# zichunhao/lgn-autoencoder

Hardware: AMD Instinct MI355X
Metric: jets/sec fwd+bwd, 30-particle maxdim=2 bs=512 (higher is better)
Workload: dtype f64

## Files before the change

### include/lgn_amd.h

```cpp
#ifndef LGN_AMD_H
#define LGN_AMD_H

#include <stddef.h>
#include <stdint.h>

#ifdef __cplusplus
extern "C" {
#endif

#define LGN_AMD_ABI_VERSION 19

int lgn_abi_version(void);
const char* lgn_last_error(void);

int lgn_level_fwd_f64(int B, int N, int C, int CO, int decoder,
                      const double* s_in, const double* v_in, const double* p, const uint8_t* mask,
                      const double* ra, const double* rb, const double* rc,
                      const double* w0, const double* b0, const double* w1, const double* b1,
                      const double* wm0, const double* wm1,
                      double* ag0, double* ag1, double* s_out, double* v_out, void* stream);

int lgn_level_bwd_partial_rows(int B, int N, int decoder, int* rows_mix, int* rows_rad);
int lgn_level_rad_partial_len(int C, int decoder);
int lgn_level_jet_split(int B, int N);

int lgn_level_bwd_f64(int B, int N, int C, int CO, int decoder,
                      const double* s_in, const double* v_in, const double* p, const uint8_t* mask,
                      const double* ra, const double* rb, const double* rc,
                      const double* w0, const double* b0, const double* w1, const double* b1,
                      const double* wm0, const double* wm1, const double* ag0, const double* ag1,
                      const double* g_s_out, const double* g_v_out,
                      double* g_ag, double* g_s_in, double* g_v_in, double* g_p,
                      double* part_mix, double* part_rad, void* stream);

int lgn_cg_product_fwd_f64(int R, int N, int C, int D1, int D2, int DO, int mode, int nnz, const int* row_ptr, const int* col,
                           const double* coef, const double* x1, const double* x2, double* out, void* stream);
int lgn_cg_product_bwd_f64(int R, int N, int C, int D1, int D2, int DO, int mode, int nnz, const int* row_ptr, const int* col,
                           const double* coef, const double* x1, const double* x2, const double* g_out, double* g_x1, double* g_x2,
                           void* stream);

int lgn_reduce_partials_f64(const double* part, int rows, int n, double* out, int accumulate, void* stream);

int lgn_radial_finalize_f64(const double* tot, int C, const double* ra, const double* rb, const double* rc,
                            const double* w0, const double* w1,
                            double* g_a, double* g_b, double* g_c,
                            double* g_w0, double* g_b0, double* g_w1, double* g_b1, void* stream);

#define LGN_ACT_LEAKYRELU 0
#define LGN_ACT_RELU 1
#define LGN_ACT_ELU 2
#define LGN_ACT_SIGMOID 3
#define LGN_ACT_LOGSIGMOID 4
#define LGN_ACT_ATAN 5
#define LGN_ACT_COUNT 6
int lgn_cgmlp_fwd_f64(int M, int C, int H, int nlin, int activation, const double* const* w, const double* const* b,
                      const double* s_in, double* s_out, void* stream);
int lgn_cgmlp_partial_rows(int M, int H);
int lgn_cgmlp_bwd_f64(int M, int C, int H, int nlin, int activation, const double* const* w, const double* const* b,
                      const double* s_in, const double* g_out, double* g_in, double* part, int psize, void* stream);

int lgn_mixreps_fwd_f64(int rows, int Cin, int Cout, int d, const double* w, const double* x, double* y, void* stream);
int lgn_mixreps_partial_rows(int rows);
int lgn_mixreps_bwd_f64(int rows, int Cin, int Cout, int d, const double* w, const double* x, const double* g_y,
                        double* g_x, double* part, void* stream);

int lgn_moments_fwd_f64(int B, int N, int C, int Q, int decoder, const double* X, const double* p, const uint8_t* mask,
                        const double* ra, const double* rb, const double* rc, const double* w0, const double* b0,
                        const double* w1, const double* b1, double* U, void* stream);
long long lgn_moments_scratch_doubles(int B, int N, int C, int decoder);
int lgn_moments_bwd_f64(int B, int N, int C, int Q, int decoder, const double* X, const double* p, const uint8_t* mask,
                        const double* ra, const double* rb, const double* rc, const double* w0, const double* b0,
                        const double* w1, const double* b1, const double* gU, double* gX, double* g_p,
                        double* part_rad, double* scratch, void* stream);

typedef struct lgn_local_tables {
  int n_rows, n_out, n_w;
  int n_terms, n_u, n_x;
  int n_units, static_kind;
  const int *row_ptr, *t_type, *t_a, *t_b;
  const double* t_coef;
  const int *out_dim, *out_nblk, *out_row0, *out_q0, *out_w0;
  const int *u_ptr, *u_row;
  const double* u_coef;
  const int *x_ptr, *x_row, *x_other;
  const double* x_coef;
  int h_out_w0[8];
} lgn_local_tables;

int lgn_local_fwd_f64(int nodes, int C, int CO, int Q, int Qout, const lgn_local_tables* t, const double* X, const double* U,
                      const double* wcat, double* out, void* stream);
int lgn_local_partial_rows(int nodes);
int lgn_local_bwd_f64(int nodes, int C, int CO, int Q, int Qout, const lgn_local_tables* t, const double* X, const double* U,
                      const double* wcat, const double* g_out, double* gU, double* gX, double* part, void* stream);

long long lgn_local_static_packed_doubles(int kind, int C, int CO);
int lgn_local_bwd_static_f64(int kind, int nodes, int C, int CO, const double* XT, const double* UT, const double* wcat,
                             const int* w0, double* wpacked, const double* goT, double* gUT, double* gXT, double* part,
                             double* gpacked, double* g_wcat, void* stream);
int lgn_local_fwd_static_f64(int kind, int nodes, int C, int CO, const double* XT, const double* UT, const double* wcat,
                             const int* w0, double* wpacked, double* outT, double* s_copy, int q_s, void* stream);

typedef struct lgn_net_desc {
  int B, N;
  int n_levels;
  int enc_channels[5];
  int dec_channels[5];
  int tau_s, tau_v;
  int mlp_hidden_mul;
  int mlp_nlin;
  int tau_v_in;
  const lgn_local_tables* enc_tables[4];
  const lgn_local_tables* dec_tables[4];
  int enc_Q[5], enc_qs[5], enc_qv[5];
  int dec_Q[5], dec_qs[5], dec_qv[5];
  int flags;
  int activation;
  int n_in_scalars;
  int latent_pool;
  int dec_N;
  int get_real;
  double jet_loss_scale;
} lgn_net_desc;
#define LGN_REAL_SUM 0
#define LGN_REAL_REAL 1
#define LGN_REAL_IMAG 2
#define LGN_REAL_MEAN 3
#define LGN_REAL_NORM 4
#define LGN_LOSS_CHAMFER 0
#define LGN_LOSS_MSE 1
#define LGN_LOSS_HUNGARIAN 2
typedef struct lgn_loss_desc {
  int kind;
  int abs_coord;
  int polar_coord;
  double scale;
} lgn_loss_desc;
#define LGN_POOL_MIN 0
#define LGN_POOL_MAX 1
#define LGN_POOL_MEAN 2
#define LGN_POOL_MIX 3
#define LGN_POOL(n, avg, o0, o1, o2, o3) ((n) | ((avg) << 3) | ((o0) << 4) | ((o1) << 6) | ((o2) << 8) | ((o3) << 10))
#define LGN_NET_NO_STATIC 1
#define LGN_NET_DEC_PAIRWISE 2
#define LGN_NET_LEVEL_V2 4
#define LGN_NET_MLP_V1 8
#define LGN_NET_MOMENTS_V1 16
#define LGN_NET_BWD_ORDERED 64
#define LGN_NET_DEC_UNFUSED 256
#define LGN_NET_MOMENTS_SPLIT 512
#define LGN_NET_MLP_BWD1 1024
#define LGN_NET_SPLIT_TAIL 128

#define LGN_LDS_LIMIT (160 * 1024)
long long lgn_encoder_end_lds_bytes(int N, int C0, int K, int CL, int Ts, int Tv, int pool);
long long lgn_decoder_end_lds_bytes(int N, int C0, int Tin, int CL);
long long lgn_junction_lds_bytes(int N, int CL, int Ts, int Tv, int pool, int C0);

int lgn_step_param_slots(const lgn_net_desc* d, int decoder);
long long lgn_step_workspace_doubles(const lgn_net_desc* d);
int lgn_step_fwd_bwd_f64(const lgn_net_desc* d, const double* params, double* grads, long long n_params,
                         const int64_t* enc_off, const int64_t* dec_off, const double* p4, const double* target,
                         const uint8_t* mask, const double* in_scalars, double* workspace, long long workspace_doubles,
                         double* recon, double* loss_part, const lgn_loss_desc* loss, int* assignment ,
                         int* status , void* stream);
#define LGN_FINALIZE_SCRATCH 2048
int lgn_step_finalize_f64(double* params, double* grads, long long n_params, const double* loss_part, int n_loss,
                          double l1_lambda, double* adam_m, double* adam_v, long long* step_dev,
                          double lr, double beta1, double beta2, double eps, int do_adam, double* loss_out, void* stream);
int lgn_step_train_f64(const lgn_net_desc* d, double* params, double* grads, long long n_params, const int64_t* enc_off,
                       const int64_t* dec_off, const double* p4, const double* target, const uint8_t* mask, const double* in_scalars,
                       double* workspace, long long workspace_doubles, double* recon, double* loss_part, int n_loss, double l1_lambda,
                       double* adam_m, double* adam_v, long long* step_dev, double lr, double beta1, double beta2, double eps,
                       int do_adam, double* loss_out, const lgn_loss_desc* loss, int* assignment ,
                       int* status , void* stream);

#define LGN_OPT_ADAM 0
#define LGN_OPT_RMSPROP 1
typedef struct {
  int kind;
  double l1_lambda, l2_lambda, lr, eps;
  double beta1, beta2;
  double alpha, momentum;
} lgn_optim_desc;
#define LGN_FINALIZE_OPT_SCRATCH 4096
int lgn_step_finalize_opt_f64(double* params, double* grads, long long n_params, const double* loss_part, int n_loss,
                              const lgn_optim_desc* opt, double* state_m, double* state_v, long long* step_dev, int do_step,
                              double* loss_out, void* stream);
int lgn_step_train_opt_f64(const lgn_net_desc* d, double* params, double* grads, long long n_params, const int64_t* enc_off,
                           const int64_t* dec_off, const double* p4, const double* target, const uint8_t* mask,
                           const double* in_scalars, double* workspace, long long workspace_doubles, double* recon,
                           double* loss_part, int n_loss, const lgn_optim_desc* opt, double* state_m, double* state_v,
                           long long* step_dev, int do_step, double* loss_out, const lgn_loss_desc* loss,
                           int* assignment , int* status , void* stream);

long long lgn_eval_workspace_doubles(const lgn_net_desc* d);
int lgn_step_eval_f64(const lgn_net_desc* d, const double* params, const int64_t* enc_off, const int64_t* dec_off,
                      const double* p4_scaled, const double* p4_target, const uint8_t* mask, const double* in_scalars,
                      double* workspace, long long workspace_doubles, double* recon_real, double* lat_s ,
                      double* lat_v , double* loss_part, double* loss_out, const lgn_loss_desc* loss,
                      int* assignment , int* status , void* stream);

long long lgn_net_workspace_doubles(const lgn_net_desc* d, int decoder, int which);
int lgn_encoder_fwd_f64(const lgn_net_desc* d, const double* params, const int64_t* off, const double* p4, const uint8_t* mask,
                        const double* in_scalars, double* act, long long act_doubles, double* lat_s, double* lat_v, void* stream);
int lgn_encoder_bwd_f64(const lgn_net_desc* d, const double* params, double* grads, long long n_params, const int64_t* off,
                        const double* p4, const uint8_t* mask, const double* in_scalars, const double* act, long long act_doubles,
                        const double* g_lat_s, const double* g_lat_v, double* scratch, long long scratch_doubles, void* stream);
int lgn_decoder_fwd_f64(const lgn_net_desc* d, const double* params, const int64_t* off, const double* lat_v, double* act,
                        long long act_doubles, double* recon, void* stream);
int lgn_decoder_bwd_f64(const lgn_net_desc* d, const double* params, double* grads, long long n_params, const int64_t* off,
                        const double* lat_v, const double* act, long long act_doubles, const double* g_recon, double* g_lat_v,
                        double* scratch, long long scratch_doubles, void* stream);

int lgn_chamfer_f64(int B, int N, int M, const double* x, const double* y, int jet_features, double* loss_part, double* gx, double* gy,
                    void* stream);

#define LGN_ANOMALY_NMAX 192
#define LGN_ANOMALY_NSCORES 21
#define LGN_ANOMALY_ALL 0x1FFFFF
#define LGN_ANOMALY_HUNGARIAN 0x403E0
#define LGN_ANOMALY_NO_HUNGARIAN (LGN_ANOMALY_ALL & ~LGN_ANOMALY_HUNGARIAN)
int lgn_anomaly_scores_f64(const double* recons, const double* target, const double* recons_n, const double* target_n, int B, int N,
                           int score_mask, double* scores, int* col4row , int* status, void* stream);

#define LGN_ROC_TILE 2048
#define LGN_ROC_MAX_COLS 65535
#define LGN_ROC_NONFINITE 1
#define LGN_ROC_SINGLE_CLASS 2
#define LGN_ROC_BAD_LABEL 4
#define LGN_ROC_NAN 8
long long lgn_roc_workspace_bytes(long long M, int K);
int lgn_roc_auc_f64(const double* scores, long long M, int ld, int K, const double* labels, double* fpr, double* tpr,
                    double* thresholds, int* length, double* auc, int* flipped, int* status, void* workspace,
// ... 113 lines not shown
```

### lgn-autoencoder_amd/csrc/api.hip

```cpp
#include "net.hpp"

using namespace lgn;

extern "C" {

int lgn_level_fwd_f64(int B, int N, int C, int CO, int decoder, const double* s_in, const double* v_in, const double* p,
                      const uint8_t* mask, const double* ra, const double* rb, const double* rc, const double* w0,
                      const double* b0, const double* w1, const double* b1, const double* wm0, const double* wm1,
                      double* ag0, double* ag1, double* s_out, double* v_out, void* stream) {
  LGN_CHECK_ARG(s_in && v_in && p && b0 && b1 && wm0 && wm1 && ag0 && ag1 && s_out && v_out, "level_fwd: null pointer");
  LGN_CHECK_ARG(decoder || (mask && ra && rb && rc && w0 && w1), "level_fwd: encoder needs mask and radial parameters");
  LevelArgs<double> a{B, N, C, CO, s_in, v_in, p, mask, ra, rb, rc, w0, b0, w1, b1, wm0, wm1, ag0, ag1, s_out, v_out};
  a.flags = level_flags_from_env();
  return level_fwd_dispatch<double>(a, decoder, (hipStream_t)stream);
}

int lgn_level_bwd_partial_rows(int B, int N, int decoder, int* rows_mix, int* rows_rad) {
  LGN_CHECK_ARG(B > 0 && N > 0 && rows_mix && rows_rad, "level_bwd_partial_rows: bad arguments");
  level_bwd_partial_rows(B, N, decoder, level_flags_from_env(), rows_mix, rows_rad);
  return 0;
}

int lgn_level_rad_partial_len(int C, int decoder) { return rad_partial_size(C, decoder != 0); }
int lgn_level_jet_split(int B, int N) { return N <= 40 ? level_jet_split(B, N) : 1; }

int lgn_level_bwd_f64(int B, int N, int C, int CO, int decoder, const double* s_in, const double* v_in, const double* p,
                      const uint8_t* mask, const double* ra, const double* rb, const double* rc, const double* w0,
                      const double* b0, const double* w1, const double* b1, const double* wm0, const double* wm1,
                      const double* ag0, const double* ag1, const double* g_s_out, const double* g_v_out, double* g_ag,
                      double* g_s_in, double* g_v_in, double* g_p, double* part_mix, double* part_rad, void* stream) {
  LGN_CHECK_ARG(s_in && v_in && p && b0 && b1 && wm0 && wm1 && ag0 && ag1 && g_s_out && g_v_out && g_ag && g_s_in &&
                    g_v_in && part_mix && part_rad, "level_bwd: null pointer");
  LGN_CHECK_ARG(decoder ? (g_p != nullptr) : (mask && ra && rb && rc && w0 && w1), "level_bwd: missing decoder g_p / encoder radial parameters");
  LevelBwdArgs<double> a{B, N, C, CO, s_in, v_in, p, mask, ra, rb, rc, w0, b0, w1, b1, wm0, wm1, ag0, ag1,
                         g_s_out, g_v_out, g_ag, g_s_in, g_v_in, g_p, part_mix, part_rad};
  a.flags = level_flags_from_env();
  return level_bwd_dispatch<double>(a, decoder, (hipStream_t)stream);
}

int lgn_cg_product_fwd_f64(int R, int N, int C, int D1, int D2, int DO, int mode, int nnz, const int* row_ptr, const int* col,
                           const double* coef, const double* x1, const double* x2, double* out, void* stream) {
  return cg_product_fwd(R, N, C, D1, D2, DO, mode, nnz, row_ptr, col, coef, x1, x2, out, (hipStream_t)stream);
}
int lgn_cg_product_bwd_f64(int R, int N, int C, int D1, int D2, int DO, int mode, int nnz, const int* row_ptr, const int* col,
                           const double* coef, const double* x1, const double* x2, const double* g_out, double* g_x1, double* g_x2,
                           void* stream) {
  return cg_product_bwd(R, N, C, D1, D2, DO, mode, nnz, row_ptr, col, coef, x1, x2, g_out, g_x1, g_x2, (hipStream_t)stream);
}

int lgn_reduce_partials_f64(const double* part, int rows, int n, double* out, int accumulate, void* stream) {
  LGN_CHECK_ARG(part && out && rows > 0 && n >= 0, "reduce_partials: bad arguments");
  return reduce_partials<double>(part, rows, n, out, accumulate, (hipStream_t)stream);
}

int lgn_radial_finalize_f64(const double* tot, int C, const double* ra, const double* rb, const double* rc, const double* w0,
                            const double* w1, double* g_a, double* g_b, double* g_c, double* g_w0, double* g_b0,
                            double* g_w1, double* g_b1, void* stream) {
  LGN_CHECK_ARG(tot && ra && rb && rc && w0 && w1 && g_a && g_b && g_c && g_w0 && g_b0 && g_w1 && g_b1 && C >= 1 && C <= 8,
                "radial_finalize: bad arguments");
  return rad_finalize<double>(tot, C, ra, rb, rc, w0, w1, g_a, g_b, g_c, g_w0, g_b0, g_w1, g_b1, (hipStream_t)stream);
}

static int fill_mlp(MlpArgs<double>& a, int M, int C, int H, int nlin, int activation, const double* const* w, const double* const* b) {
  LGN_CHECK_ARG(nlin >= 1 && nlin <= MLP_MAX_LIN && w && b, "cgmlp: bad layer list (nlin=%d)", nlin);
  a.M = M; a.C = C; a.H = H; a.nlin = nlin; a.act = activation;
  for (int l = 0; l < MLP_MAX_LIN; ++l) {
    a.w[l] = l < nlin ? w[l] : nullptr;
    a.b[l] = l < nlin ? b[l] : nullptr;
    if (l < nlin) LGN_CHECK_ARG(w[l] && b[l], "cgmlp: null weight pointer for layer %d", l);
  }
  return 0;
}

int lgn_cgmlp_fwd_f64(int M, int C, int H, int nlin, int activation, const double* const* w, const double* const* b,
                      const double* s_in, double* s_out, void* stream) {
  MlpArgs<double> a{};
  if (int rc = fill_mlp(a, M, C, H, nlin, activation, w, b)) return rc;
  LGN_CHECK_ARG(s_in && s_out, "cgmlp_fwd: null pointer");
  a.s_in = s_in; a.s_out = s_out;
  a.flags = level_flags_from_env();
  return mlp_dispatch<double>(a, false, (hipStream_t)stream);
}

int lgn_cgmlp_partial_rows(int M, int H) { return mlp_partial_rows(M, H); }

int lgn_cgmlp_bwd_f64(int M, int C, int H, int nlin, int activation, const double* const* w, const double* const* b,
                      const double* s_in, const double* g_out, double* g_in, double* part, int psize, void* stream) {
  MlpArgs<double> a{};
  if (int rc = fill_mlp(a, M, C, H, nlin, activation, w, b)) return rc;
  LGN_CHECK_ARG(s_in && g_out && g_in && part, "cgmlp_bwd: null pointer");
  a.s_in = s_in; a.g_out = g_out; a.g_in = g_in; a.part = part; a.psize = psize;
  a.flags = level_flags_from_env();
  return mlp_dispatch<double>(a, true, (hipStream_t)stream);
}

int lgn_mixreps_fwd_f64(int rows, int Cin, int Cout, int d, const double* w, const double* x, double* y, void* stream) {
  LGN_CHECK_ARG(w && x && y, "mixreps_fwd: null pointer");
// ... 253 lines not shown
```

### lgn-autoencoder_amd/csrc/api_common.cpp

```cpp
#include <stdarg.h>
#include <stdlib.h>

#include "level.hpp"
#include "../../include/lgn_amd.h"

namespace lgn {
static thread_local char g_err[512] = "";
void set_error(const char* fmt, ...) {
  va_list ap;
  va_start(ap, fmt);
  vsnprintf(g_err, sizeof(g_err), fmt, ap);
  va_end(ap);
}
int level_flags_from_env() {
  auto on = [](const char* name) { const char* e = getenv(name); return e && e[0] == '1'; };
  return (on("LGN_AMD_DEC_PAIRWISE") ? LVL_DEC_PAIRWISE : 0) | (on("LGN_AMD_LEVEL_V2") ? LVL_LEVEL_V2 : 0) |
         (on("LGN_AMD_MOMENTS_V1") ? LVL_MOMENTS_V1 : 0) | (on("LGN_AMD_MLP_V1") ? LVL_MLP_V1 : 0) | (on("LGN_AMD_BWD_ORDERED") ? LVL_BWD_ORDERED : 0) |
         (on("LGN_AMD_MOMENTS_SPLIT") ? LVL_MOMENTS_SPLIT : 0) | (on("LGN_AMD_MLP_BWD1") ? LVL_MLP_BWD1 : 0);
}
static_assert(LVL_DEC_PAIRWISE == LGN_NET_DEC_PAIRWISE && LVL_LEVEL_V2 == LGN_NET_LEVEL_V2 && LVL_MOMENTS_V1 == LGN_NET_MOMENTS_V1 &&
                  LVL_MLP_V1 == LGN_NET_MLP_V1 && LVL_MLP_BWD1 == LGN_NET_MLP_BWD1 &&
                  LVL_BWD_ORDERED == LGN_NET_BWD_ORDERED && LVL_MOMENTS_SPLIT == LGN_NET_MOMENTS_SPLIT, "LVL_* and LGN_NET_* are the same bits");
}

extern "C" {
const char* lgn_last_error(void) { return lgn::g_err; }
int lgn_abi_version(void) { return LGN_AMD_ABI_VERSION; }
}
```

### lgn-autoencoder_amd/csrc/level.hpp

```cpp
#pragma once
#include "common.hpp"

namespace lgn {

constexpr int LVL_DEC_PAIRWISE = 2;
constexpr int LVL_LEVEL_V2 = 4;
constexpr int LVL_MLP_V1 = 8;
constexpr int LVL_MOMENTS_V1 = 16;
constexpr int LVL_MLP_BWD1 = 1024;
constexpr int LVL_MOMENTS_SPLIT = 512;
constexpr int LVL_BWD_ORDERED = 64;
int level_flags_from_env();

template <typename T>
struct LevelArgs {
  int B, N, C, CO;
  const T* s_in;
  const T* v_in;
  const T* p;
  const uint8_t* mask;
  const T *ra, *rb, *rc, *w0, *b0, *w1, *b1;
  const T *wm0, *wm1;
  T* ag0;
  T* ag1;
  T* s_out;
  T* v_out;
  const T* in_w0 = nullptr;
  const T* in_w1 = nullptr;
  T* in_s = nullptr;
  T* in_v = nullptr;
  T* z1 = nullptr;
  size_t z1n = 0;
  T* z2 = nullptr;
  size_t z2n = 0;
  const T* loss_wo1 = nullptr;
  const T* loss_target = nullptr;
  T loss_scale = T(1);
  int loss_real = 0;
  T loss_jscale = T(0);
  T* loss_recon = nullptr;
  T* loss_part = nullptr;
  T* loss_gv = nullptr;
  T* loss_wpart = nullptr;
  int flags = 0;
};

template <typename T>
struct LevelBwdArgs {
  int B, N, C, CO;
  const T *s_in, *v_in, *p;
  const uint8_t* mask;
  const T *ra, *rb, *rc, *w0, *b0, *w1, *b1;
  const T *wm0, *wm1;
  const T *ag0, *ag1;
  const T* g_s_out;
  const T* g_v_out;
  T* g_ag;
  T* g_s_in;
  T* g_v_in;
  T* g_p;
  T* part_mix;
  T* part_rad;
  T* part_in0 = nullptr;
  int flags = 0;
};

__host__ __device__ constexpr int node_stride(int C) { return 10 * C + 4; }

__host__ __device__ constexpr int rad_partial_size(int C, bool dec) {
  return dec ? 2 * C : (2 * 4 * C * NB + 8 * C);
}

inline int level_jet_split(int B, int N) {
  const int groups = (N + 3) / 4;
  int s = 1;
  while (s * 2 <= groups && B * s * 2 <= 512) s *= 2;
  return s;
}

}
```

### lgn-autoencoder_amd/csrc/level_bwd3.hip

```cpp
#include "level_dev.hpp"
#include "ops.hpp"
#include "wave_sum.hpp"

namespace lgn {

typedef double v4d __attribute__((ext_vector_type(4)));

namespace {
__device__ __forceinline__ double dppq(double v, int xor2) {
  int lo = __double2loint(v), hi = __double2hiint(v);
  if (xor2) {
    lo = __builtin_amdgcn_mov_dpp(lo, 0x4E, 0xF, 0xF, true);
    hi = __builtin_amdgcn_mov_dpp(hi, 0x4E, 0xF, 0xF, true);
  } else {
    lo = __builtin_amdgcn_mov_dpp(lo, 0xB1, 0xF, 0xF, true);
    hi = __builtin_amdgcn_mov_dpp(hi, 0xB1, 0xF, 0xF, true);
  }
  return __hiloint2double(hi, lo);
}
__device__ __forceinline__ double quad_sum(double v) {
  v += dppq(v, 0);
  v += dppq(v, 1);
  return v;
}
__device__ __forceinline__ double fast_rcp(double u) {
  double r = __builtin_amdgcn_rcp(u);
  double e = __builtin_fma(-u, r, 1.0);
  r = __builtin_fma(r, e, r);
  e = __builtin_fma(-u, r, 1.0);
  return __builtin_fma(r, e, r);
}
__device__ __forceinline__ void wave_sync() {
  __builtin_amdgcn_fence(__ATOMIC_RELEASE, "workgroup");
  __builtin_amdgcn_wave_barrier();
  __builtin_amdgcn_fence(__ATOMIC_ACQUIRE, "workgroup");
}
template <int C> struct GA3 {
  static constexpr int A3 = 0, A4 = 2 * C, A1 = 4 * C, A2 = 12 * C, SIZE = 20 * C + 2;
};
constexpr int TS = 18;
LGN_STAMP_DECL
}
LGN_STAMP_READER(lgn_debug_stamps_bwd3)

template <int C, bool DEC, int NWV = 4>
struct Bwd3 {
  static constexpr int BLK = 64 * NWV;
  static constexpr int NG = (C + 3) / 4;
  static constexpr int NS = node_stride(C);
  static constexpr int PS = DEC ? 8 : 4;
  static constexpr int TRSZ = DEC ? NWV * 64 : (NWV * (NG + 3) * 16 * TS > NWV * 64 * NG * 12 ? NWV * (NG + 3) * 16 * TS : NWV * 64 * NG * 12);
  static constexpr int MIXP = BLK / (5 * C) < 16 ? BLK / (5 * C) : 16;
  __host__ __device__ static size_t scratch(int N, int CO) {
    size_t p1 = (size_t)N * 10 * CO + 4 * CO * 5 * C + (size_t)N * 20 * C;
    const size_t red = (size_t)MIXP * CO * 5 * C * 4;
    if (red > p1) p1 = red;
    return p1 > (size_t)TRSZ ? p1 : (size_t)TRSZ;
  }
  static constexpr int SMS = 52;
  static constexpr int SEPSZ = DEC ? SMS * C : 0;
  static size_t smem(int N, int CO) {
    return sizeof(double) * ((((size_t)N * NS + 1) & ~size_t(1)) + (size_t)N * (20 * C + 2) + (size_t)N * 10 * C + (size_t)N * PS +
                             scratch(N, CO) + SEPSZ) + N + 16;
  }
};

template <int C, bool DEC, bool SEP, int NWV, bool SYM = false>
__global__ __launch_bounds__(64 * NWV) __attribute__((amdgpu_waves_per_eu(C <= 4 || DEC ? 2 : 1, C <= 4 || DEC ? 2 : 1))) void level_bwd3_kernel(LevelBwdArgs<double> a) {
  static_assert(!SYM || !DEC, "the symmetric sweep is the encoder's");
  using F = Bwd3<C, DEC, NWV>;
  constexpr int BLK = F::BLK;
  using G = GA3<C>;
  constexpr int NG = F::NG, NS = F::NS, PS = F::PS, K = 5 * C;
  const int N = a.N, B = a.B, CO = a.CO;
  const int b = blockIdx.x, tid = threadIdx.x, lane = tid & 63, wave = tid >> 6;
  const int ngroups = (N + 3) >> 2, gper = (ngroups + (int)gridDim.y - 1) / (int)gridDim.y;
  const int glo = min(ngroups, (int)blockIdx.y * gper), ghi = min(ngroups, glo + gper);
  const int nlo = min(N, 4 * glo), nhi = min(N, 4 * ghi);
  const size_t prow = (size_t)b * gridDim.y + blockIdx.y;

  extern __shared__ __align__(16) unsigned char smem_raw[];
  double* nd = reinterpret_cast<double*>(smem_raw);
  double* ga = nd + ((N * NS + 1) & ~1);
  double* gd = ga + N * G::SIZE;
  double* pj = gd + N * 10 * C;
  double* tr = pj + N * PS;
  double* go = tr;
  double* wm = go + N * 10 * CO;
  double* agl = wm + 4 * CO * K;
  double* sm = tr + F::scratch(N, CO);
  uint8_t* mk = reinterpret_cast<uint8_t*>(sm + F::SEPSZ);

  STAMP(0);
  {
    const size_t plo = (size_t)B * N * CO, pa = (size_t)B * N * 2 * C;
    JetRegs<double> jr;
    load_jet_issue<double, C, DEC>(a.s_in, a.v_in, a.p, a.mask, B, N, b, jr);
    const int eg = tid < N * CO ? tid : 0, ea_ = tid < N * 2 * C ? tid : 0, ew = tid < 2 * CO * K ? tid : 0;
    const size_t ig = (size_t)b * N * CO + eg, ia = (size_t)b * N * 2 * C + ea_;
    double rg[10], ra[10];
    rg[0] = a.g_s_out[ig];
    rg[1] = a.g_s_out[plo + ig];
    ra[0] = a.ag0[ia];
    ra[1] = a.ag0[pa + ia];
#pragma unroll
    for (int m = 0; m < 4; ++m) {
      rg[2 + m] = a.g_v_out[ig * 4 + m];
      rg[6 + m] = a.g_v_out[plo * 4 + ig * 4 + m];
      ra[2 + m] = a.ag1[ia * 4 + m];
      ra[6 + m] = a.ag1[(pa + ia) * 4 + m];
    }
    const double w0v = a.wm0[ew], w1v = a.wm1[ew];
    load_jet_commit<double, C, DEC>(a.s_in, a.v_in, a.p, a.mask, B, N, b, jr, nd, pj, mk);
    if (tid < N * CO) {
#pragma unroll
      for (int m = 0; m < 10; ++m) go[tid * 10 + m] = rg[m];
    }
    if (tid < N * 2 * C) {
#pragma unroll
      for (int m = 0; m < 10; ++m) agl[tid * 10 + m] = ra[m];
    }
    if (tid < 2 * CO * K) {
      wm[tid] = w0v;
      wm[2 * CO * K + tid] = w1v;
    }
    for (int e = tid + BLK; e < 2 * CO * K; e += BLK) {
      wm[e] = a.wm0[e];
      wm[2 * CO * K + e] = a.wm1[e];
    }
    for (int e = tid + BLK; e < N * CO; e += BLK) {
      const size_t idx = (size_t)b * N * CO + e;
      double* g = go + e * 10;
      g[0] = a.g_s_out[idx];
      g[1] = a.g_s_out[plo + idx];
#pragma unroll
      for (int m = 0; m < 4; ++m) {
        g[2 + m] = a.g_v_out[idx * 4 + m];
        g[6 + m] = a.g_v_out[plo * 4 + idx * 4 + m];
      }
    }
    for (int e = tid + BLK; e < N * 2 * C; e += BLK) {
      const size_t ea = (size_t)b * N * 2 * C + e;
      double* x = agl + e * 10;
      x[0] = a.ag0[ea];
      x[1] = a.ag0[pa + ea];
#pragma unroll
      for (int m = 0; m < 4; ++m) {
        x[2 + m] = a.ag1[ea * 4 + m];
        x[6 + m] = a.ag1[(pa + ea) * 4 + m];
      }
    }
  }
  __syncthreads();
  STAMP(1);

  {
    const int half = tid >= BLK / 2;
    for (int e = half ? tid - BLK / 2 : tid; e < N * C; e += BLK / 2) {
// ... 268 lines not shown
          const double* q = sm + c * F::SMS;
          const double* ni = nd + n * NS + c * 10;
          const cx<double> R1 = {a.b1[c], a.b1[c]};
          const cx<double> S = {q[0], q[1]}, SG3 = {q[22], q[23]};
          const cx<double> VSt = {sg * q[2 + 2 * mp], sg * q[3 + 2 * mp]};
          const cx<double> vt = {sg * ni[2 + mp], sg * ni[6 + mp]};
          const cx<double> g2 = {gi[G::A2 + (c * 4 + m) * 2], gi[G::A2 + (c * 4 + m) * 2 + 1]};
          const cx<double> g3 = {0.5 * gi[G::A3 + 2 * c], 0.5 * gi[G::A3 + 2 * c + 1]};
          cx<double> t = cmulc(g2, S);
          cfmac(t, g3, VSt);
          const cx<double> t2 = cmulc(cx<double>{q[32 + 2 * m], q[33 + 2 * m]}, cx<double>{ni[0], ni[1]});
          t.r -= t2.r;  t.i -= t2.i;
          const cx<double> t3 = cmulc(SG3, vt);
          t.r -= t3.r;  t.i -= t3.i;
          cfmac(acc, t, R1);
        }
        a.g_p[((size_t)b * N + n) * 4 + m] += acc.r;
        a.g_p[plp + ((size_t)b * N + n) * 4 + m] += acc.i;
      }
    }
    if (tid < 2 * C) {
      const int lin = tid / C, c = tid - lin * C;
      const double* q = sm + c * F::SMS;
      const cx<double> S = {q[0], q[1]};
      double* part = a.part_rad + (size_t)blockIdx.x * rad_partial_size(C, true);
      if (lin == 0) {
        cx<double> E0 = cmulc(cx<double>{q[20], q[21]}, S);
#pragma unroll
        for (int m = 0; m < 4; ++m) cfmac(E0, cx<double>{q[24 + 2 * m], q[25 + 2 * m]}, cx<double>{q[2 + 2 * m], q[3 + 2 * m]});
        part[tid] = (E0.r + E0.i) + (E0.i - E0.r);
      } else {
        cx<double> VS[4], VSt[4];
#pragma unroll
        for (int m = 0; m < 4; ++m) VS[m] = {q[2 + 2 * m], q[3 + 2 * m]};
        metric_perm(VS, VSt);
        cx<double> E1 = cmulc(cx<double>{q[40], q[41]}, S);
        cx<double> neg = cmulc(cx<double>{q[22], q[23]}, cx<double>{q[18], q[19]});
#pragma unroll
        for (int m = 0; m < 4; ++m) {
          cfmac(neg, cx<double>{q[32 + 2 * m], q[33 + 2 * m]}, cx<double>{q[10 + 2 * m], q[11 + 2 * m]});
          cfmac(E1, cx<double>{q[42 + 2 * m], q[43 + 2 * m]}, VSt[m]);
        }
        part[tid] = (E1.r - neg.r) + (E1.i - neg.i);
      }
    }
    STAMP(7);
    return;
  }

  STAMP(3);
  const int pr = lane & 15, cg = lane >> 4;
  const int tj = pr >> 2, ti = pr & 3;
  double ak[5], bk[5], ck2[5], wf[NG][5], bias[NG][4];
  if (!DEC) {
#pragma unroll
    for (int s = 0; s < 5; ++s) {
      const int k = 4 * s + cg;
      ak[s] = a.ra[k];
      bk[s] = a.rb[k];
      const double c = a.rc[k];
      ck2[s] = c * c;
    }
#pragma unroll
    for (int g = 0; g < NG; ++g) {
      const int rr = lane & 15, q = rr >> 2, ch = 4 * g + (rr & 3);
      const double* w = (q >> 1) ? a.w1 : a.w0;
#pragma unroll
      for (int s = 0; s < 5; ++s) wf[g][s] = ch < C ? w[(2 * ch + (q & 1)) * NB + 4 * s + cg] : 0.0;
    }
  }
#pragma unroll
  for (int g = 0; g < NG; ++g) {
    const int ch = 4 * g + cg;
#pragma unroll
    for (int q = 0; q < 4; ++q) {
      const double* bb = (q >> 1) ? a.b1 : a.b0;
      bias[g][q] = ch < C ? (DEC ? bb[ch] : bb[2 * ch + (q & 1)]) : 0.0;
    }
  }
  STAMP(4);
  __syncthreads();
  STAMP(5);

  double* trw = tr + wave * (NG + 3) * 16 * TS;
  v4d T[NG][3];
  double dB0[NG], dB1[NG];
#pragma unroll
  for (int g = 0; g < NG; ++g) {
    dB0[g] = dB1[g] = 0.0;
#pragma unroll
    for (int t = 0; t < 3; ++t) T[g][t] = v4d{0, 0, 0, 0};
  }
  const size_t pls = (size_t)B * N * C;
  double in0[NG][4];
#pragma unroll
  for (int g = 0; g < NG; ++g) in0[g][0] = in0[g][1] = in0[g][2] = in0[g][3] = 0.0;
  const int gcount = ghi - glo;
  const int rs = (!SYM && !DEC && NWV == 4 && gcount >= 1 && gcount <= 2) ? NWV / gcount : 1;
  const int rpart = rs > 1 ? wave % rs : 0;
  const int ntl = (N + 3) >> 2, i0lo = rs > 1 ? 4 * (rpart * ntl / rs) : 0, i0hi = rs > 1 ? min(N, 4 * ((rpart + 1) * ntl / rs)) : N;
  for (int u = 0;; ++u) {
    int rg;
    if constexpr (SYM) {
      const int p = wave + NWV * (u >> 1);
      if (p >= (ngroups + 1) >> 1) break;
      rg = (u & 1) ? ngroups - 1 - p : p;
      if ((u & 1) && rg == p) continue;
    } else if (rs > 1) {
      if (u > 0) break;
      rg = glo + wave / rs;
    } else {
      rg = glo + wave + NWV * u;
      if (rg >= ghi) break;
    }
    const int j = rg * 4 + tj;
    const bool jok = j < N;
    const int jj = jok ? j : N - 1;
    double pme[PS];
#pragma unroll
    for (int m = 0; m < PS; ++m) pme[m] = pj[jj * PS + m];
    const bool mj = DEC ? false : (mk[jj] != 0);
    cx<double> Gs[NG], Gv[NG][4], Gq[4];
    cx<double> sj[NG], vj[NG][4], vtj[NG][4];
    cx<double> dvj[NG], svj[NG];
#pragma unroll
    for (int g = 0; g < NG; ++g) {
      Gs[g] = {0, 0};
#pragma unroll
      for (int m = 0; m < 4; ++m) Gv[g][m] = {0, 0};
      const int ch = 4 * g + cg, cs = ch < C ? ch : 0;
      const double* nj = nd + jj * NS + cs * 10;
      sj[g] = {nj[0], nj[1]};
#pragma unroll
      for (int m = 0; m < 4; ++m) vj[g][m] = {nj[2 + m], nj[6 + m]};
      metric_perm(vj[g], vtj[g]);
      dvj[g] = {vj[g][3].r - vj[g][1].r, vj[g][3].i - vj[g][1].i};
      svj[g] = {vj[g][1].r + vj[g][3].r, vj[g][1].i + vj[g][3].i};
    }
#pragma unroll
    for (int m = 0; m < 4; ++m) Gq[m] = {0, 0};

    for (int i0 = i0lo; i0 < i0hi; i0 += 4) {
      if (rg == glo && i0 < 32) STAMP(16 + (i0 >> 2) * 4);
      const int kind = SYM ? ((i0 >> 2) < rg ? 2 : ((i0 >> 2) == rg ? 1 : 0)) : 1;
      const int i = i0 + ti;
      const bool ok = jok && i < N;
      const int ii = i < N ? i : N - 1;
      const double* pii = pj + ii * PS;
      cx<double> q[4];
      v4d R[NG];
      double rho[5], an = 0.0;
      double qd0 = 0.0, qd3 = 0.0, qa = 0.0, qb = 0.0;
      bool on = false;
      if (DEC) {
#pragma unroll
        for (int m = 0; m < 4; ++m) q[m] = {pii[m] - pme[m], pii[4 + m] - pme[4 + m]};
#pragma unroll
        for (int g = 0; g < NG; ++g) R[g] = v4d{bias[g][0], bias[g][1], bias[g][2], bias[g][3]};
      } else {
        const double d0 = pii[0] - pme[0], d1 = pii[1] - pme[1], d2 = pii[2] - pme[2], d3 = pii[3] - pme[3];
        const double q0 = d0 * d0, q1 = d1 * d1, q2 = d2 * d2, q3 = d3 * d3;
        const double nsq = (2.0 * q0 - (((q0 + q1) + q2) + q3)) + 1e-16;
        an = fabs(nsq);
        on = ok && mj && (mk[ii] != 0) && (nsq != 0.0);
        const double h = rsqrt2<double>();
        q[0] = {d0, 0.0};
        q[1] = {d1 * h, -d2 * h};
        q[2] = {d3, 0.0};
        q[3] = {-d1 * h, -d2 * h};
        qd0 = d0;  qd3 = d3;  qa = d1 * h;  qb = d2 * h;
        double beta[5] = {0.0, 0.0, 0.0, 0.0, 0.0};
#pragma unroll
        for (int s = 0; s < 5; ++s) rho[s] = 0.0;
        if (on) {
#pragma unroll
          for (int s = 0; s < 5; ++s) beta[s] = 1.0 + ck2[s] * an;
          rcp5(beta, rho);
#pragma unroll
          for (int s = 0; s < 5; ++s) beta[s] = __builtin_fma(bk[s], rho[s], ak[s]);
        }
#pragma unroll
        for (int g = 0; g < NG; ++g) {
          R[g] = v4d{bias[g][0], bias[g][1], bias[g][2], bias[g][3]};
#pragma unroll
          for (int s = 0; s < 5; ++s) R[g] = __builtin_amdgcn_mfma_f64_16x16x4f64(wf[g][s], beta[s], R[g], 0, 0, 0);
        }
        if (kind != 0) {
          double* xb = trw + NG * 16 * TS;
#pragma unroll
          for (int s = 0; s < 5; ++s) {
            const double x2 = an * rho[s] * rho[s];
            if (s < 4) {
              xb[pr * TS + 4 * s + cg] = rho[s];
              xb[16 * TS + pr * TS + 4 * s + cg] = x2;
            } else {
              xb[32 * TS + pr * TS + cg] = rho[s];
              xb[32 * TS + pr * TS + 4 + cg] = x2;
            }
          }
          xb[32 * TS + pr * TS + 8 + 2 * cg] = cg == 0 ? (on ? 1.0 : 0.0) : 0.0;
          xb[32 * TS + pr * TS + 9 + 2 * cg] = cg == 0 ? (ok ? 1.0 : 0.0) : 0.0;
        }
      }
      if (rg == glo && i0 < 32) STAMP(17 + (i0 >> 2) * 4);
      const double* gi = ga + ii * G::SIZE;
#pragma unroll
      for (int g = 0; g < NG; ++g) {
        const int ch = 4 * g + cg;
        double G0r = 0, G0i = 0, G1r = 0, G1i = 0;
        if (ok && ch < C) {
          const cx<double> R0 = {R[g][0], R[g][1]}, R1 = {R[g][2], R[g][3]};
          const cx<double> e0 = {R0.r - R0.i, R0.r + R0.i};
          const cx<double> gA3 = {0.5 * gi[G::A3 + 2 * ch], 0.5 * gi[G::A3 + 2 * ch + 1]};
          const cx<double> gA4 = {gi[G::A4 + 2 * ch], gi[G::A4 + 2 * ch + 1]};
          cx<double> gA1[4], gA2[4];
#pragma unroll
          for (int m = 0; m < 4; ++m) {
            gA1[m] = {gi[G::A1 + (ch * 4 + m) * 2], gi[G::A1 + (ch * 4 + m) * 2 + 1]};
            gA2[m] = {gi[G::A2 + (ch * 4 + m) * 2], gi[G::A2 + (ch * 4 + m) * 2 + 1]};
          }
          cfmac(Gs[g], gA4, e0);
          cx<double> ge0 = cmulc(gA4, sj[g]);
          cx<double> gR1;
          if (!DEC) {
            const cx<double> dg = {gA2[1].r - gA2[3].r, gA2[1].i - gA2[3].i}, sg = {gA2[1].r + gA2[3].r, gA2[1].i + gA2[3].i};
// ... 237 lines not shown
  if constexpr (!DEC) {
    if (a.part_in0) {
#pragma unroll
      for (int g = 0; g < NG; ++g)
#pragma unroll
        for (int k = 0; k < 4; ++k) {
          double x = in0[g][k];
          x += shfl_xor(x, 4);
          x += shfl_xor(x, 8);
          if (pr == 0 && 4 * g + cg < C) in0l[wave][4 * g + cg][k] = x;
        }
    }
  }

  STAMP(8);
  __syncthreads();
  STAMP(9);
  if constexpr (!DEC) {
    if (a.part_in0 && tid < 4 * C) {
      const int k = tid / C, c = tid - k * C;
      double s = 0;
#pragma unroll
      for (int w = 0; w < NWV; ++w) s += in0l[w][c][k];
      a.part_in0[prow * 4 * C + k * C + c] = s;
    }
  }
  double* part = a.part_rad + prow * rad_partial_size(C, DEC);
  if (DEC) {
    double* red = tr;
#pragma unroll
    for (int g = 0; g < NG; ++g) {
      double x0 = dB0[g], x1 = dB1[g];
      for (int m = 1; m < 16; m <<= 1) { x0 += shfl_xor(x0, m); x1 += shfl_xor(x1, m); }
      if (pr == 0) {
        red[(wave * NG + g) * 8 + cg] = x0;
        red[(wave * NG + g) * 8 + 4 + cg] = x1;
      }
    }
    __syncthreads();
    if (tid < 2 * C) {
      const int lin = tid / C, ch = tid - lin * C, g = ch >> 2, c4 = ch & 3;
      double s = 0;
      for (int w = 0; w < NWV; ++w) s += red[(w * NG + g) * 8 + lin * 4 + c4];
      part[tid] = s;
    }
  } else {
    double* red = tr;
    {
      double* mine = red + (size_t)(wave * 64 + lane) * NG * 12;
#pragma unroll
      for (int g = 0; g < NG; ++g)
#pragma unroll
        for (int t = 0; t < 3; ++t)
#pragma unroll
          for (int q = 0; q < 4; ++q) mine[(g * 3 + t) * 4 + q] = T[g][t][q];
    }
    __syncthreads();
    const int wq = __builtin_amdgcn_readfirstlane(wave);
    if (wq < 4) {
      constexpr int R = 4 * C;
      const int col = lane & 15;
#pragma unroll
      for (int g = 0; g < NG; ++g) {
        const int ch = 4 * g + cg;
#pragma unroll
        for (int t = 0; t < 3; ++t)
#pragma unroll
          for (int q = 0; q < 4; ++q) {
            if (q != wq) continue;
            const int e = (g * 3 + t) * 4 + q;
            double v = (red[(size_t)(0 * 64 + lane) * NG * 12 + e] + red[(size_t)(1 * 64 + lane) * NG * 12 + e]) +
                       (red[(size_t)(2 * 64 + lane) * NG * 12 + e] + red[(size_t)(3 * 64 + lane) * NG * 12 + e]);
            if (NWV == 8)
              v += (red[(size_t)(4 * 64 + lane) * NG * 12 + e] + red[(size_t)(5 * 64 + lane) * NG * 12 + e]) +
                   (red[(size_t)(6 * 64 + lane) * NG * 12 + e] + red[(size_t)(7 * 64 + lane) * NG * 12 + e]);
            if (ch >= C) continue;
            const int r = (q >> 1) * 2 * C + 2 * ch + (q & 1);
            if (t == 0) part[r * NB + col] = v;
            else if (t == 1) part[R * NB + r * NB + col] = v;
            else {
              if (col < 4) part[r * NB + 16 + col] = v;
              else if (col < 8) part[R * NB + r * NB + 16 + (col - 4)] = v;
              else if (col == 8) part[2 * R * NB + r] = v;
              else if (col == 9) part[2 * R * NB + R + r] = v;
            }
          }
      }
    }
  }
  STAMP(10);
}

bool level_bwd3_fits(int N) { return N <= 40; }

template <int C, bool DEC, bool SEP, int NWV>
static int launch_bwd3_w(const LevelBwdArgs<double>& a, int split, hipStream_t stream) {
  size_t smem = Bwd3<C, DEC, NWV>::smem(a.N, a.CO);
  LGN_CHECK_ARG(smem <= 160 * 1024, "level_bwd: N=%d C=%d needs %zu B of LDS", a.N, a.C, smem);
  LGN_CHECK_ARG(a.CO <= 8, "level_bwd: C_out=%d unsupported (1..8)", a.CO);
  auto kern = level_bwd3_kernel<C, DEC, SEP, NWV>;
  if constexpr (!DEC && C <= 4) {
    if (split == 1 && !(a.flags & LVL_BWD_ORDERED)) kern = level_bwd3_kernel<C, DEC, SEP, NWV, true>;
  }
  if (smem > 64 * 1024) (void)hipFuncSetAttribute(reinterpret_cast<const void*>(kern), hipFuncAttributeMaxDynamicSharedMemorySize, (int)smem);
  hipLaunchKernelGGL(kern, dim3(a.B, split), dim3(64 * NWV), smem, stream, a);
  LGN_CHECK_LAUNCH();
  return 0;
}
template <int C, bool DEC, bool SEP>
static int launch_bwd3(const LevelBwdArgs<double>& a, hipStream_t stream) {
  return launch_bwd3_w<C, DEC, SEP, 4>(a, SEP ? 1 : level_jet_split(a.B, a.N), stream);
}

int level_bwd3_dispatch(const LevelBwdArgs<double>& a, int decoder, hipStream_t stream) {
  const bool pairwise = (a.flags & LVL_DEC_PAIRWISE) != 0;
#define LGN_CASE(CC)                                                                \
  case CC:                                                                          \
    if (!decoder) return launch_bwd3<CC, false, false>(a, stream);                  \
    return pairwise ? launch_bwd3<CC, true, false>(a, stream) : launch_bwd3<CC, true, true>(a, stream);
  switch (a.C) {
#ifdef LGN_DEV_ONLY_C4
    LGN_CASE(4)
#else
    LGN_CASE(1) LGN_CASE(2) LGN_CASE(3) LGN_CASE(4) LGN_CASE(5) LGN_CASE(6) LGN_CASE(7) LGN_CASE(8)
#endif
    default: set_error("level_bwd: C_in=%d unsupported (1..8)", a.C); return -1;
  }
#undef LGN_CASE
}

}
```

### lgn-autoencoder_amd/csrc/level_fwd2.hip

```cpp
#include "level_dev.hpp"
#include "net_dev.hpp"
#include "ops.hpp"
#include "wave_sum.hpp"

namespace lgn {

typedef double v4d __attribute__((ext_vector_type(4)));
LGN_STAMP_DECL
LGN_STAMP_READER(lgn_debug_stamps_fwd2)

__device__ __forceinline__ double dpp_quad(double v, int ctrl_is_xor2) {
  int lo = __double2loint(v), hi = __double2hiint(v);
  if (ctrl_is_xor2) {
    lo = __builtin_amdgcn_mov_dpp(lo, 0x4E, 0xF, 0xF, true);
    hi = __builtin_amdgcn_mov_dpp(hi, 0x4E, 0xF, 0xF, true);
  } else {
    lo = __builtin_amdgcn_mov_dpp(lo, 0xB1, 0xF, 0xF, true);
    hi = __builtin_amdgcn_mov_dpp(hi, 0xB1, 0xF, 0xF, true);
  }
  return __hiloint2double(hi, lo);
}
__device__ __forceinline__ double quad_sum(double v) {
  v += dpp_quad(v, 0);
  v += dpp_quad(v, 1);
  return v;
}

__device__ __forceinline__ double fast_rcp(double u) {
  double r = __builtin_amdgcn_rcp(u);
  double e = __builtin_fma(-u, r, 1.0);
  r = __builtin_fma(r, e, r);
  e = __builtin_fma(-u, r, 1.0);
  return __builtin_fma(r, e, r);
}

template <int C, bool DEC>
struct Fwd2 {
  static constexpr int NG = (C + 3) / 4;
  static constexpr int NS = node_stride(C);
  static constexpr int PS = DEC ? 8 : 4;
  static constexpr int AGS = 20 * C;
  static constexpr int A3 = 0, A4 = 2 * C, A1 = 4 * C, A2 = 12 * C;
};

template <int C, bool DEC, bool SEP, bool TRAIN>
__global__ __launch_bounds__(2 * BLOCK) void level_fwd2_kernel(LevelArgs<double> a, int chunk) {
  using F = Fwd2<C, DEC>;
  constexpr int NG = F::NG;
  const int N = a.N, B = a.B, CO = a.CO;
  const int b = blockIdx.x, tid = threadIdx.x, lane = tid & 63, wave = tid >> 6;
  const int nthr = blockDim.x, nw = nthr >> 6;

  extern __shared__ __align__(16) unsigned char smem_raw[];
  double* nd = reinterpret_cast<double*>(smem_raw);
  double* pj = nd + ((N * F::NS + 1) & ~1);
  double* wm = pj + N * F::PS;
  double* agl = wm + 4 * CO * 5 * C;
  double* sums = agl + chunk * F::AGS;
  uint8_t* mk = reinterpret_cast<uint8_t*>(sums + 20 * C);

  STAMP(0);
  if (!DEC && a.in_w0) {
    {
      const size_t wg = (size_t)blockIdx.y * gridDim.x + blockIdx.x, stride = (size_t)gridDim.x * gridDim.y * nthr;
      for (size_t e = wg * nthr + tid; e < a.z1n; e += stride) a.z1[e] = 0.0;
      for (size_t e = wg * nthr + tid; e < a.z2n; e += stride) a.z2[e] = 0.0;
    }
    const double* p0 = a.p + (size_t)b * N * 4;
    const size_t plane_s = (size_t)B * N * C;
    const int nw2 = 2 * CO * 5 * C;
    for (int e = tid; e < N * 4; e += nthr) pj[e] = p0[e];
    for (int e = tid; e < N; e += nthr) mk[e] = a.mask[(size_t)b * N + e];
    for (int e = tid; e < nw2; e += nthr) {
      wm[e] = a.wm0[e];
      wm[nw2 + e] = a.wm1[e];
    }
    for (int e = tid; e < N * C; e += nthr) {
      const int j = e / C, c = e - j * C;
      const double* p = p0 + j * 4;
      const double pe = p[0], px = p[1], py = p[2], pz = p[3];
      const double q0 = pe * pe, q1 = px * px, q2 = py * py, q3 = pz * pz;
      const double mass = sqrt(fabs(2.0 * q0 - (((q0 + q1) + q2) + q3)));
      constexpr double H = 0.70710678118654752440084436210484903928;
      const cx<double> q[4] = {{pe, 0.0}, {px * H, -py * H}, {pz, 0.0}, {-px * H, -py * H}};
      const double w0r = a.in_w0[c], w0i = a.in_w0[C + c];
      const cx<double> w1 = {a.in_w1[c], a.in_w1[C + c]};
      double* d = nd + j * F::NS + c * 10;
      d[0] = w0r * mass;
      d[1] = w0i * mass;
#pragma unroll
      for (int m = 0; m < 4; ++m) {
        const cx<double> r = cmul(w1, q[m]);
        d[2 + m] = r.r;
        d[6 + m] = r.i;
      }
      if (blockIdx.y == 0) {
        const size_t ge = (size_t)b * N * C + e;
        a.in_s[ge] = d[0];
        a.in_s[plane_s + ge] = d[1];
#pragma unroll
        for (int m = 0; m < 4; ++m) {
          a.in_v[ge * 4 + m] = d[2 + m];
          a.in_v[plane_s * 4 + ge * 4 + m] = d[6 + m];
        }
      }
    }
  } else {
    JetRegs<double> jr;
    load_jet_issue<double, C, DEC>(a.s_in, a.v_in, a.p, a.mask, B, N, b, jr);
    const int nw2 = 2 * CO * 5 * C, ew = tid < nw2 ? tid : 0;
    const double w0v = a.wm0[ew], w1v = a.wm1[ew];
    load_jet_commit<double, C, DEC>(a.s_in, a.v_in, a.p, a.mask, B, N, b, jr, nd, pj, mk);
    if (tid < nw2) {
      wm[tid] = w0v;
      wm[nw2 + tid] = w1v;
    }
    for (int e = tid + nthr; e < nw2; e += nthr) {
      wm[e] = a.wm0[e];
      wm[nw2 + e] = a.wm1[e];
    }
  }

  const int pr = lane & 15, cg = lane >> 4;
  const int ti = pr >> 2, tj = pr & 3;
  double ak[5], bk[5], ck2[5];
  double wf[NG][5];
  double bias[NG][4];
  if (!DEC) {
#pragma unroll
    for (int s = 0; s < 5; ++s) {
      const int k = 4 * s + cg;
      ak[s] = a.ra[k];
      bk[s] = a.rb[k];
      const double c = a.rc[k];
      ck2[s] = c * c;
    }
#pragma unroll
    for (int g = 0; g < NG; ++g) {
      const int rr = lane & 15, q = rr >> 2, ch = 4 * g + (rr & 3);
      const double* w = (q >> 1) ? a.w1 : a.w0;
#pragma unroll
      for (int s = 0; s < 5; ++s) wf[g][s] = ch < C ? w[(2 * ch + (q & 1)) * NB + 4 * s + cg] : 0.0;
    }
  }
#pragma unroll
  for (int g = 0; g < NG; ++g) {
    const int ch = 4 * g + cg;
#pragma unroll
    for (int q = 0; q < 4; ++q) {
      const double* bb = (q >> 1) ? a.b1 : a.b0;
      bias[g][q] = ch < C ? (DEC ? bb[ch] : bb[2 * ch + (q & 1)]) : 0.0;
    }
  }
  __syncthreads();
  STAMP(1);

  if constexpr (DEC && SEP) {
    if (tid < 64) {
      const int k = tid & 7, part = tid >> 3;
      double mean = 0.0;
      for (int n = part; n < N; n += 8) mean += pj[n * 8 + k];
      mean += shfl_xor(mean, 8);
      mean += shfl_xor(mean, 16);
      mean += shfl_xor(mean, 32);
      if (part == 0) sums[k] = mean / N;
    }
    __syncthreads();
    for (int e = tid; e < N * 8; e += nthr) pj[e] -= sums[e & 7];
    __syncthreads();
#define LGN_PUT(k, val)                                           \
  do {                                                            \
    if ((k) < 12) a0[(k) < 12 ? (k) : 0] += (val);                \
    else a1[(k) >= 12 ? (k) - 12 : 0] += (val);                   \
  } while (0)
    for (int c = wave; c < C; c += nw) {
      double a0[12], a1[8];
#pragma unroll
      for (int k = 0; k < 12; ++k) a0[k] = 0.0;
#pragma unroll
      for (int k = 0; k < 8; ++k) a1[k] = 0.0;
      for (int n = lane; n < N; n += 64) {
        const double* ni = nd + n * F::NS + c * 10;
        const double* pn = pj + n * 8;
        const cx<double> sn = {ni[0], ni[1]};
        cx<double> v[4], pc[4];
#pragma unroll
        for (int m = 0; m < 4; ++m) {
          v[m] = {ni[2 + m], ni[6 + m]};
          pc[m] = {pn[m], pn[4 + m]};
        }
        LGN_PUT(0, sn.r);  LGN_PUT(1, sn.i);
#pragma unroll
        for (int m = 0; m < 4; ++m) {
          LGN_PUT(2 + 2 * m, v[m].r);  LGN_PUT(3 + 2 * m, v[m].i);
          const cx<double> sp = cmul(sn, pc[m]);
          LGN_PUT(10 + 2 * m, sp.r);  LGN_PUT(11 + 2 * m, sp.i);
        }
        const cx<double> vp = bil2(v, pc);
        LGN_PUT(18, vp.r);  LGN_PUT(19, vp.i);
      }
      wave_sum_store<12>(a0, sums + c * 20, lane);
      wave_sum_store<8>(a1, sums + c * 20 + 12, lane);
    }
#undef LGN_PUT
    __syncthreads();
  }

  const int ngroups = (N + 3) >> 2, gper = (ngroups + (int)gridDim.y - 1) / (int)gridDim.y;
  const int rlo = min(N, 4 * (int)blockIdx.y * gper), rhi = min(N, rlo + 4 * gper);
  auto catmix = [&](int c0, int c1) {
    constexpr int K = 5 * C;
    const int nr = c1 - c0;
    const size_t plo = (size_t)B * N * CO;
    if (wave == 0) {
      for (int rl = lane; rl < nr; rl += 64) {
        const int r = c0 + rl;
        const double* st = agl + rl * F::AGS;
        const double* ni = nd + r * F::NS;
        cx<double> x[K];
#pragma unroll
        for (int c = 0; c < C; ++c) {
          const cx<double> sc = {ni[c * 10], ni[c * 10 + 1]};
          cx<double> v[4];
#pragma unroll
          for (int mm = 0; mm < 4; ++mm) v[mm] = {ni[c * 10 + 2 + mm], ni[c * 10 + 6 + mm]};
          cx<double> vv = bil2(v, v);
          vv.r *= 0.5;  vv.i *= 0.5;
          x[c] = {st[F::A3 + 2 * c], st[F::A3 + 2 * c + 1]};
          x[C + c] = {st[F::A4 + 2 * c], st[F::A4 + 2 * c + 1]};
          x[2 * C + c] = sc;
          x[3 * C + c] = vv;
          x[4 * C + c] = cmul(sc, sc);
        }
#pragma unroll 2
        for (int o = 0; o < CO; ++o) {
          const double* wr = wm + (0 * CO + o) * K;
          const double* wi = wm + (1 * CO + o) * K;
          cx<double> acc = {0, 0};
#pragma unroll
          for (int k = 0; k < K; ++k) cfma(acc, cx<double>{wr[k], wi[k]}, x[k]);
          const size_t e = ((size_t)b * N + r) * CO + o;
          a.s_out[e] = acc.r;
          a.s_out[plo + e] = acc.i;
        }
      }
    } else {
      for (int it = lane + 64 * (wave - 1); it < nr * 4; it += 64 * (nw - 1)) {
        const int rl = it >> 2, m = it & 3, r = c0 + rl;
        const double* st = agl + rl * F::AGS;
        const double* ni = nd + r * F::NS;
        cx<double> x[K];
#pragma unroll
        for (int c = 0; c < C; ++c) {
          const cx<double> sc = {ni[c * 10], ni[c * 10 + 1]};
          const cx<double> v = {ni[c * 10 + 2 + m], ni[c * 10 + 6 + m]};
          x[c] = {st[F::A1 + (c * 4 + m) * 2], st[F::A1 + (c * 4 + m) * 2 + 1]};
          x[C + c] = {st[F::A2 + (c * 4 + m) * 2], st[F::A2 + (c * 4 + m) * 2 + 1]};
          x[2 * C + c] = v;
          x[3 * C + c] = x[4 * C + c] = cmul(v, sc);
        }
#pragma unroll 2
        for (int o = 0; o < CO; ++o) {
          const double* wr = wm + 2 * CO * K + (0 * CO + o) * K;
          const double* wi = wm + 2 * CO * K + (1 * CO + o) * K;
          cx<double> acc = {0, 0};
#pragma unroll
          for (int k = 0; k < K; ++k) cfma(acc, cx<double>{wr[k], wi[k]}, x[k]);
          const size_t e = ((size_t)b * N + r) * CO + o;
          a.v_out[e * 4 + m] = acc.r;
          a.v_out[plo * 4 + e * 4 + m] = acc.i;
        }
      }
    }
    };
  for (int c0 = rlo; c0 < rhi; c0 += chunk) {
  const int c1 = min(rhi, c0 + chunk);
  if constexpr (DEC && SEP) {
    for (int e = tid; e < (c1 - c0) * C; e += nthr) {
      const int rl = e / C, c = e - rl * C, n = c0 + rl;
      const double* sm = sums + c * 20;
      const double* pn = pj + n * 8;
      const cx<double> R0 = {a.b0[c], a.b0[c]}, R1 = {a.b1[c], a.b1[c]};
      const cx<double> e0 = {R0.r - R0.i, R0.r + R0.i};
      const cx<double> S = {sm[0], sm[1]};
      cx<double> VS[4], pc[4];
#pragma unroll
      for (int m = 0; m < 4; ++m) {
        VS[m] = {sm[2 + 2 * m], sm[3 + 2 * m]};
        pc[m] = {pn[m], pn[4 + m]};
      }
      double* st = agl + rl * F::AGS;
      const cx<double> a4 = cmul(S, e0);
// ... 43 lines not shown
      int jj;
      bool ok;
    };
    auto prep = [&](int j0, Tile& T) {
      const int j = j0 + tj;
      T.ok = iok && j < N;
      T.jj = j < N ? j : N - 1;
      const double* pjj = pj + T.jj * F::PS;
      if (DEC) {
#pragma unroll
        for (int m = 0; m < 4; ++m) T.q[m] = {pi[m] - pjj[m], pi[4 + m] - pjj[4 + m]};
#pragma unroll
        for (int g = 0; g < NG; ++g) T.R[g] = v4d{bias[g][0], bias[g][1], bias[g][2], bias[g][3]};
      } else {
        const double d0 = pi[0] - pjj[0], d1 = pi[1] - pjj[1], d2 = pi[2] - pjj[2], d3 = pi[3] - pjj[3];
        const double q0 = d0 * d0, q1 = d1 * d1, q2 = d2 * d2, q3 = d3 * d3;
        const double nsq = (2.0 * q0 - (((q0 + q1) + q2) + q3)) + 1e-16;
        const double an = fabs(nsq);
        const bool on = T.ok && mi && (mk[T.jj] != 0) && (nsq != 0.0);
        const double h = rsqrt2<double>();
        T.qd0 = d0;  T.qd3 = d3;  T.qa = d1 * h;  T.qb = d2 * h;
        double beta[5] = {0.0, 0.0, 0.0, 0.0, 0.0};
        if (on) {
#pragma unroll
          for (int s = 0; s < 5; ++s) beta[s] = 1.0 + ck2[s] * an;
          double rho5[5];
          rcp5(beta, rho5);
#pragma unroll
          for (int s = 0; s < 5; ++s) beta[s] = __builtin_fma(bk[s], rho5[s], ak[s]);
        }
#pragma unroll
        for (int g = 0; g < NG; ++g) {
          T.R[g] = v4d{bias[g][0], bias[g][1], bias[g][2], bias[g][3]};
#pragma unroll
          for (int s = 0; s < 5; ++s) T.R[g] = __builtin_amdgcn_mfma_f64_16x16x4f64(wf[g][s], beta[s], T.R[g], 0, 0, 0);
        }
      }
    };
    auto agg = [&](const Tile& T) {
      if (T.ok) {
        const double* nj = nd + T.jj * F::NS;
#pragma unroll
        for (int g = 0; g < NG; ++g) {
          const int ch = 4 * g + cg;
          if (ch < C) {
            const cx<double> R0 = {T.R[g][0], T.R[g][1]}, R1 = {T.R[g][2], T.R[g][3]};
            const cx<double> e0 = {R0.r - R0.i, R0.r + R0.i};
            const cx<double> sj = {nj[ch * 10], nj[ch * 10 + 1]};
            cx<double> vj[4];
#pragma unroll
            for (int m = 0; m < 4; ++m) {
              vj[m] = {nj[ch * 10 + 2 + m], nj[ch * 10 + 6 + m]};
              cfma(A1[g][m], vj[m], e0);
            }
            cfma(A4[g], sj, e0);
            if (!DEC) {
              const double qd0 = T.qd0, qd3 = T.qd3, qa = T.qa, qb = T.qb;
              const cx<double> Tm = cmul(sj, R1);
              A2[g][0].r = __builtin_fma(Tm.r, qd0, A2[g][0].r);  A2[g][0].i = __builtin_fma(Tm.i, qd0, A2[g][0].i);
              A2[g][2].r = __builtin_fma(Tm.r, qd3, A2[g][2].r);  A2[g][2].i = __builtin_fma(Tm.i, qd3, A2[g][2].i);
              const double aTr = qa * Tm.r, aTi = qa * Tm.i, bTr = qb * Tm.r, bTi = qb * Tm.i;
              A2[g][1].r += aTr + bTi;  A2[g][1].i += aTi - bTr;
              A2[g][3].r += bTi - aTr;  A2[g][3].i -= aTi + bTr;
              const cx<double> dv = {vj[3].r - vj[1].r, vj[3].i - vj[1].i}, sv = {vj[1].r + vj[3].r, vj[1].i + vj[3].i};
              cx<double> V;
              V.r = __builtin_fma(vj[0].r, qd0, __builtin_fma(-vj[2].r, qd3, __builtin_fma(qa, dv.r, qb * sv.i)));
              V.i = __builtin_fma(vj[0].i, qd0, __builtin_fma(-vj[2].i, qd3, __builtin_fma(qa, dv.i, -qb * sv.r)));
              cfma(A3[g], R1, V);
            } else {
              cx<double> e1[4];
#pragma unroll
              for (int m = 0; m < 4; ++m) {
                e1[m] = cmul(R1, T.q[m]);
                cfma(A2[g][m], sj, e1[m]);
              }
              const cx<double> t = bil2(vj, e1);
              A3[g].r += t.r;
              A3[g].i += t.i;
            }
          }
        }
      }
    };
    if (jlo < jhi) {
      Tile ta, tb;
      prep(jlo, ta);
      int j0 = jlo;
      while (true) {
        if (j0 + 4 < jhi) prep(j0 + 4, tb);
        agg(ta);
        j0 += 4;
        if (j0 >= jhi) break;
        if (j0 + 4 < jhi) prep(j0 + 4, ta);
        agg(tb);
        j0 += 4;
        if (j0 >= jhi) break;
      }
    }

    STAMP(3 + ((rg >> 2) & 3) * 4);
#pragma unroll
    for (int g = 0; g < NG; ++g) {
      A3[g].r = quad_sum(A3[g].r) * 0.5;  A3[g].i = quad_sum(A3[g].i) * 0.5;
      A4[g].r = quad_sum(A4[g].r);        A4[g].i = quad_sum(A4[g].i);
#pragma unroll
      for (int m = 0; m < 4; ++m) {
        A1[g][m].r = quad_sum(A1[g][m].r);  A1[g][m].i = quad_sum(A1[g][m].i);
        A2[g][m].r = quad_sum(A2[g][m].r);  A2[g][m].i = quad_sum(A2[g][m].i);
      }
    }
    if (tj == 0) {
      double* st = agl + (slab + i0 + ti - c0) * F::AGS;
#pragma unroll
      for (int g = 0; g < NG; ++g) {
        const int ch = 4 * g + cg;
        if (ch < C) {
          st[F::A3 + 2 * ch] = A3[g].r;  st[F::A3 + 2 * ch + 1] = A3[g].i;
          st[F::A4 + 2 * ch] = A4[g].r;  st[F::A4 + 2 * ch + 1] = A4[g].i;
#pragma unroll
          for (int m = 0; m < 4; ++m) {
            st[F::A1 + (ch * 4 + m) * 2] = A1[g][m].r;  st[F::A1 + (ch * 4 + m) * 2 + 1] = A1[g][m].i;
            st[F::A2 + (ch * 4 + m) * 2] = A2[g][m].r;  st[F::A2 + (ch * 4 + m) * 2 + 1] = A2[g][m].i;
          }
        }
      }
    }
    STAMP(4 + ((rg >> 2) & 3) * 4);
  };
  if (rs > 1) {
    const int rg = (c0 >> 2) + wave / rs;
    if (rg * 4 < c1) row_group(rg, 4 * (rpart * ntl / rs), min(N, 4 * ((rpart + 1) * ntl / rs)), rpart * 4 * ngr);
  } else {
    for (int rg = (c0 >> 2) + wave; rg * 4 < c1; rg += nw) row_group(rg, 0, N, 0);
  }
  if (rs > 1) {
    __syncthreads();
    const int tot = 4 * ngr * F::AGS;
    for (int e = tid; e < tot; e += nthr) {
      double v = agl[e];
      for (int pp = 1; pp < rs; ++pp) v += agl[pp * tot + e];
      agl[e] = v;
    }
  }
  }
  __syncthreads();
  STAMP(20);

  if constexpr (TRAIN) {
    const size_t pl0 = (size_t)B * N * 2 * C;
    for (int e = tid; e < (c1 - c0) * 2 * C; e += nthr) {
      const int n = e / (2 * C), r = e - n * 2 * C, blk = r / C, ch = r - blk * C;
      const double* st = agl + n * F::AGS + (blk ? F::A4 : F::A3) + 2 * ch;
      const size_t ge = ((size_t)b * N + c0) * 2 * C + e;
      a.ag0[ge] = st[0];
      a.ag0[pl0 + ge] = st[1];
    }
    for (int e = tid; e < (c1 - c0) * 2 * C * 4; e += nthr) {
      const int n = e / (8 * C), r = e - n * 8 * C, blk = r / (4 * C), cm = r - blk * 4 * C;
      const double* st = agl + n * F::AGS + (blk ? F::A2 : F::A1) + 2 * cm;
      const size_t ge = ((size_t)b * N + c0) * 8 * C + e;
      a.ag1[ge] = st[0];
      a.ag1[pl0 * 4 + ge] = st[1];
    }
  }
  STAMP(21);

  catmix(c0, c1);
  STAMP(22);
  if (c1 < rhi) __syncthreads();
  }
  STAMP(40);
  if constexpr (DEC) {
    if (a.loss_wo1) {
      __syncthreads();
      dec_output_loss_body<TRAIN>(B, N, CO, a.v_out, a.loss_wo1, a.loss_target, a.loss_scale, a.loss_real, a.loss_jscale,
                                  a.loss_recon, a.loss_part, a.loss_gv, a.loss_wpart, smem_raw);
    }
  }
}

template <int C, bool DEC, bool SEP, bool TRAIN>
static int launch_level_fwd2(const LevelArgs<double>& a, hipStream_t stream) {
  using F = Fwd2<C, DEC>;
  const size_t fixed = sizeof(double) * (((size_t)a.N * F::NS + 1 & ~size_t(1)) + (size_t)a.N * F::PS + 4 * a.CO * 5 * C + 20 * C) + a.N + 16;
  const bool wide = a.B <= 320 && a.N >= 64;
  const size_t row = sizeof(double) * F::AGS, budget1 = 160 * 1024, budget2 = wide ? budget1 : 78 * 1024;
  const int full = (a.N + 15) & ~15;
  int chunk = full;
  if (fixed + full * row > budget2) {
    const size_t room = fixed + 16 * row <= budget2 ? budget2 - fixed : (fixed < budget1 ? budget1 - fixed : 0);
    chunk = (int)(room / row) & ~15;
    if (chunk > full) chunk = full;
    if (chunk < 16) chunk = 16;
  }
  size_t smem = fixed + chunk * row;
  if (a.loss_wo1) {
    LGN_CHECK_ARG(DEC && SEP && a.N <= 40 && !wide && a.loss_target && a.loss_recon && a.loss_part && (!TRAIN || (a.loss_gv && a.loss_wpart)),
                  "level_fwd: the loss rides on the separable decoder forward of jets of <= 40 particles only");
    if (smem < dec_out_loss_bytes(a.N, a.CO)) smem = dec_out_loss_bytes(a.N, a.CO);
  }
  LGN_CHECK_ARG(smem <= 160 * 1024, "level_fwd: N=%d C=%d needs %zu B of LDS (> 160 KiB)", a.N, a.C, smem);
  auto kern = level_fwd2_kernel<C, DEC, SEP, TRAIN>;
  if (smem > 64 * 1024) {
    hipError_t e = hipFuncSetAttribute(reinterpret_cast<const void*>(kern), hipFuncAttributeMaxDynamicSharedMemorySize, (int)smem);
    if (e != hipSuccess) { set_error("hipFuncSetAttribute: %s", hipGetErrorString(e)); return (int)e; }
  }
  const int nthreads = wide ? 2 * BLOCK : BLOCK;
  const int split = (SEP || a.N > 40) ? 1 : level_jet_split(a.B, a.N);
  hipLaunchKernelGGL(kern, dim3(a.B, split), dim3(nthreads), smem, stream, a, chunk);
  LGN_CHECK_LAUNCH();
  return 0;
}

bool level_fwd_carries_loss(int N, int flags) { return N <= 40 && !(flags & LVL_DEC_PAIRWISE); }

template <bool TRAIN>
static int level_fwd_run(const LevelArgs<double>& a, int decoder, hipStream_t stream) {
  LGN_CHECK_ARG(a.B > 0 && a.N > 0, "level_fwd: empty batch (B=%d N=%d)", a.B, a.N);
  LGN_CHECK_ARG(!a.in_w0 || (!decoder && a.in_w1 && a.in_s && a.in_v), "level_fwd: the input stage rides on encoder levels only");
  LGN_CHECK_ARG(a.CO >= 1 && a.CO <= 8, "level_fwd: C_out=%d unsupported (1..8)", a.CO);
  const bool pairwise = (a.flags & LVL_DEC_PAIRWISE) != 0;
#define LGN_CASE(CC)                                                                                         \
  case CC:                                                                                                   \
    if (!decoder) return launch_level_fwd2<CC, false, false, TRAIN>(a, stream);                              \
    return pairwise ? launch_level_fwd2<CC, true, false, TRAIN>(a, stream) : launch_level_fwd2<CC, true, true, TRAIN>(a, stream);
  switch (a.C) {
#ifdef LGN_DEV_ONLY_C4
    LGN_CASE(4)
#else
    LGN_CASE(1) LGN_CASE(2) LGN_CASE(3) LGN_CASE(4) LGN_CASE(5) LGN_CASE(6) LGN_CASE(7) LGN_CASE(8)
#endif
    default:
      set_error("level_fwd: C_in=%d unsupported (1..8)", a.C);
      return -1;
  }
#undef LGN_CASE
}

template <>
int level_fwd_dispatch<double>(const LevelArgs<double>& a, int decoder, hipStream_t stream) {
  return level_fwd_run<true>(a, decoder, stream);
}

int level_fwd_eval(const LevelArgs<double>& a, int decoder, hipStream_t stream) { return level_fwd_run<false>(a, decoder, stream); }

}
```

### lgn-autoencoder_amd/csrc/ops.hpp

```cpp
#pragma once
#include <cstdlib>
#include <vector>
#include "level.hpp"

namespace lgn {

template <typename T> int level_fwd_dispatch(const LevelArgs<T>&, int decoder, hipStream_t);
int level_fwd_eval(const LevelArgs<double>&, int decoder, hipStream_t);
template <typename T> int level_bwd_dispatch(const LevelBwdArgs<T>&, int decoder, hipStream_t);
template <typename T> int reduce_partials(const T* part, int rows, int n, T* out, int accumulate, hipStream_t);
template <typename T> int reduce_partials_strided(const T* part, int rows, int stride, int col0, int n, T* out, hipStream_t);
constexpr int RED_MAX_SEG = 64;
template <typename T> struct RedSeg { const T* part; int rows, stride, col0, n; T* out; };
template <typename T> struct RedJob {
  int nseg;
  RedSeg<T> seg[RED_MAX_SEG];
  int tile0[RED_MAX_SEG + 1];
  void add(const T* part, int rows, int stride, int col0, int n, T* out) { seg[nseg++] = RedSeg<T>{part, rows, stride, col0, n, out}; }
};
template <typename T> int reduce_segments(RedJob<T>& job, hipStream_t);
template <typename T>
int rad_finalize(const T* tot, int C, const T* ra, const T* rb, const T* rc, const T* w0, const T* w1, T* g_a, T* g_b, T* g_c,
                 T* g_w0, T* g_b0, T* g_w1, T* g_b1, hipStream_t);
struct RadFinJob {
  int n;
  struct Item { const double* tot; int C; const double *ra, *rb, *rc, *w0, *w1; double *g_a, *g_b, *g_c, *g_w0, *g_b0, *g_w1, *g_b1; } it[4];
};
int rad_finalize_batch(const RadFinJob& job, hipStream_t);
struct StepTailArgs {
  double *w, *g;
  long n;
  double *m, *v;
  long* step_dev;
  double lambda, lr, beta1, beta2, eps;
  int do_adam;
  const double* loss_part;
  int nB;
  double* loss_out;
  int reduce_only;
  unsigned long long* counters;
  int opt_form = 0;
  int kind = 0;
  double l2 = 0.0, alpha = 0.0, mu = 0.0;
};
int step_tail(const std::vector<RedSeg<double>>& segs, const RadFinJob& fin, const StepTailArgs& ta, hipStream_t st);
void level_bwd_partial_rows(int B, int N, int decoder, int flags, int* rows_mix, int* rows_rad);
bool level_bwd_carries_input(int N, int flags);
bool level_fwd_carries_loss(int N, int flags);

constexpr int MLP_MAX_LIN = 8;
template <typename T>
struct MlpArgs {
  int M;
  int C;
  int H;
  int nlin;
  const T* w[MLP_MAX_LIN];
  const T* b[MLP_MAX_LIN];
  const T* s_in;
  T* s_out;
  const T* g_out;
  T* g_in;
  T* part;
  int psize;
  int ld = 1;
  int tbQ = 0;
  T* h_saved = nullptr;
  int h_rows = 0;
  int act = 0;
  int flags = 0;
};
inline int mlp_saved_rows(int M) { return (M + 63) & ~63; }
inline size_t mlp_saved_doubles(int M, int H, int nlin) {
  return H <= 48 && nlin >= 4 && nlin <= 7 ? (size_t)(nlin - 1) * mlp_saved_rows(M) * ((H + 15) & ~15) : 0;
}
constexpr int MLP_SAVE_MAX_ROWS = 8128;
inline size_t mlp_save_max_rows() {
  static const long v = [] { const char* e = getenv("LGN_AMD_MLP_SAVE_ROWS"); return e ? atol(e) : (long)MLP_SAVE_MAX_ROWS; }();
  return (size_t)(v < 0 ? 0 : v);
}
template <typename T>
__host__ __device__ inline size_t mlp_out_index(const MlpArgs<T>& a, int z, int row, int ch) {
  if (a.tbQ > 0) return ((size_t)((row >> 6) * a.C + ch) * a.tbQ) * 128 + z * 64 + (row & 63);
  return ((size_t)z * a.M * a.C + (size_t)row * a.C + ch) * a.ld;
}
template <typename T> int mlp_dispatch(const MlpArgs<T>&, bool backward, hipStream_t);
int cg_product_fwd(int R, int N, int C, int D1, int D2, int DO, int mode, int nnz, const int* row_ptr, const int* col, const double* coef,
                   const double* x1, const double* x2, double* out, hipStream_t st);
int cg_product_bwd(int R, int N, int C, int D1, int D2, int DO, int mode, int nnz, const int* row_ptr, const int* col, const double* coef,
                   const double* x1, const double* x2, const double* g_out, double* g_x1, double* g_x2, hipStream_t st);
int mlp_mfma_dispatch(const MlpArgs<double>&, bool backward, hipStream_t);
int mlp_chain_dispatch(const MlpArgs<double>&, bool backward, hipStream_t);
int mlp_mfma_wide_dispatch(const MlpArgs<double>&, bool backward, hipStream_t);
inline int mlp_rows_per_workgroup(int M, int H) { return (H <= 48 && (M + 63) / 64 < 128) ? 16 : 64; }
inline int mlp_partial_rows(int M, int H) { const int r = mlp_rows_per_workgroup(M, H); return (M + r - 1) / r; }

template <typename T>
struct MixArgs {
  int rows, Cin, Cout, d;
  const T* w;
  const T* x;
  T* y;
  const T* g_y;
  T* g_x;
  T* part;
};
template <typename T> int mix_fwd(const MixArgs<T>&, hipStream_t);
template <typename T> int mix_bwd(const MixArgs<T>&, hipStream_t);
int mix_partial_rows(int rows);

struct GenArgs {
  int B, N, C, Q;
  const double* X;
  const double* p;
  const uint8_t* mask;
  const double *ra, *rb, *rc, *w0, *b0, *w1, *b1;
  double* U;
  const double* gU;
  double* gX;
  double* g_p;
  double* part_rad;
  double* gbuf;
  int flags;
  int tb;
};
__host__ __device__ inline size_t feat_index(bool tb, size_t plane, int C, int Qx, int n, int c, int q, int z) {
  return tb ? ((size_t)((n >> 6) * C + c) * Qx + q) * 128 + z * 64 + (n & 63) : (size_t)z * plane + ((size_t)n * C + c) * Qx + q;
}
size_t moments2_gbuf_doubles(int B, int N, int C);
int moments_dispatch(const GenArgs& a, int decoder, int which, hipStream_t st);
// ... 75 lines not shown
```

### lgn-autoencoder_amd/csrc/step.hip

```cpp
#include <stdlib.h>

#include <algorithm>
#include <mutex>
#include <vector>

#include "net.hpp"
#include "../../include/lgn_amd.h"

namespace lgn {
namespace {

struct Bump {
  double* base;
  size_t off = 0;
  double* take(size_t n) {
    n = (n + 15) & ~size_t(15);
    double* p = base ? base + off : nullptr;
    off += n;
    return p;
  }
};

struct NetBuf {
  double *s[5], *v[5], *smix[4], *ag0[4], *ag1[4];
  double* hsave[4];
};

struct Work {
  NetBuf enc, dec;
  double *lat_s, *lat_v, *pdec, *g_lat_s, *g_lat_v, *g_p;
  double *gs[2], *gv[2], *gsmix, *g_ag, *zeros_s;
  double *parts;
  size_t parts_size;
  double* tot[2][4];
  int* idx;
  size_t total;
  double* tail_cnt;
  double* zero0() const { return tail_cnt < zeros_s ? tail_cnt : zeros_s; }
  size_t zero_doubles;
};

struct Deferred {
  std::vector<RedSeg<double>> segs;
  double* parts;
  size_t off = 0, cap = 0;
  double* take(size_t n) {
    n = (n + 15) & ~size_t(15);
    if (off + n > cap) return nullptr;
    double* p = parts + off;
    off += n;
    return p;
  }
  void add(const double* part, int rows, int stride, int col0, int n, double* out) {
    if (n > 0) segs.push_back(RedSeg<double>{part, rows, stride, col0, n, out});
  }
  int flush(hipStream_t st) {
    for (size_t i = 0; i < segs.size(); i += RED_MAX_SEG) {
      RedJob<double> job{};
      for (size_t k = i; k < segs.size() && k < i + RED_MAX_SEG; ++k) job.seg[job.nseg++] = segs[k];
      if (int rc = reduce_segments<double>(job, st)) return rc;
    }
    segs.clear();
    return 0;
  }
};

int finish_reductions(Deferred& dq, const RadFinJob& fin, double* grads, long long n_params, double* counters, int flags, hipStream_t st) {
  if (counters && !(flags & LGN_NET_SPLIT_TAIL)) {
    StepTailArgs ro{};
    ro.g = grads;
    ro.n = (long)n_params;
    ro.reduce_only = 1;
    ro.counters = reinterpret_cast<unsigned long long*>(counters);
    const int rc = step_tail(dq.segs, fin, ro, st);
    if (rc == 0) { dq.segs.clear(); return 0; }
    if (rc != -2) return rc;
  }
  if (int rc = dq.flush(st)) return rc;
  return rad_finalize_batch(fin, st);
}

int finalize_tail(const StepTailArgs& t, hipStream_t st) {
  if (t.opt_form) return finalize_step_opt(t, st);
  return finalize_step(t.w, t.g, t.n, t.loss_part, t.nB, t.lambda, t.m, t.v, t.step_dev, t.lr, t.beta1, t.beta2, t.eps, t.do_adam,
                       t.loss_out, st);
}

int end_step(Deferred& dq, const RadFinJob& fin, double* grads, long long n_params, double* counters, int flags, const StepTailArgs* tail,
             hipStream_t st) {
  if (tail && !(flags & LGN_NET_SPLIT_TAIL)) {
    const int rc = step_tail(dq.segs, fin, *tail, st);
    if (rc != -2) return rc;
  }
  if (int rc = finish_reductions(dq, fin, grads, n_params, tail ? nullptr : counters, flags, st)) return rc;
  if (!tail) return 0;
  return finalize_tail(*tail, st);
}

inline int in_K(const lgn_net_desc& d) { return d.n_in_scalars > 1 ? d.n_in_scalars : 1; }

int mlp_psize(int C, int H, int nlin) {
  const int D = 2 * C;
  return nlin == 1 ? D * D + D : (H * D + H) + (nlin - 2) * (H * H + H) + (D * H + D);
}

inline int dec_nodes(const lgn_net_desc& d) { return d.dec_N > 0 ? d.dec_N : d.N; }
inline bool step_is_split(const lgn_net_desc& d) { return dec_nodes(d) != d.N || d.n_in_scalars > 1; }
inline int dec_tin(const lgn_net_desc& d) { return d.tau_v_in > 0 ? d.tau_v_in : pool_blocks(d.latent_pool) * d.tau_v; }
int check_latent_match(const lgn_net_desc& d) {
  const int Tin = pool_blocks(d.latent_pool) * d.tau_v;
  LGN_CHECK_ARG(d.tau_v_in == 0 || d.tau_v_in == Tin, "step: the decoder must consume the encoder's %d pooled latent vectors", Tin);
  return 0;
}

struct Slots {
  int L, nlin;
  int in0(bool dec) const { return dec ? 2 : 0; }
  int rad(bool dec, int l, int k) const { return in0(dec) + 2 + 7 * l + k; }
// ... 6 lines not shown
struct RowLayout {
  int width, nseg, col[3], n[3], slot[3];
  void add(Deferred& dq, const double* part, int rows, double* G, const int64_t* off) const {
    for (int i = 0; i < nseg; ++i) dq.add(part, rows, width, col[i], n[i], G + off[slot[i]]);
  }
};
RowLayout enc_latent_rows(const lgn_net_desc& d, int N, int CL) {
  const int KL = pool_mix_in(d.latent_pool, N, CL), o = Slots{d.n_levels, d.mlp_nlin}.out0(false);
  return {2 * (d.tau_s + d.tau_v) * KL, 2, {0, 2 * d.tau_s * KL}, {2 * d.tau_s * KL, 2 * d.tau_v * KL}, {o, o + 1}};
}
RowLayout enc_input_rows(int K, int C0) { return {(2 * K + 2) * C0, 2, {0, 2 * C0 * K}, {2 * C0 * K, 2 * C0}, {0, 1}}; }
RowLayout dec_input_rows(int C0, int N, int Tin) {
  return {4 * C0 + 2 * N * Tin, 3, {0, 2 * C0, 4 * C0}, {2 * C0, 2 * C0, 2 * N * Tin}, {2, 3, 1}};
}
RowLayout dec_output_rows(const lgn_net_desc& d, int CL) {
  return {2 * CL, 1, {0}, {2 * CL}, {Slots{d.n_levels, d.mlp_nlin}.out0(true) + 1}};
}

inline size_t r16(size_t n) { return (n + 15) & ~size_t(15); }
size_t end_parts(const lgn_net_desc& d, bool dec, int N, int in_rows) {
  const int* ch = dec ? d.dec_channels : d.enc_channels;
  const int L = d.n_levels;
  if (dec) return r16((size_t)d.B * dec_output_rows(d, ch[L]).width) + r16((size_t)d.B * dec_input_rows(ch[0], N, dec_tin(d)).width);
  return r16((size_t)d.B * enc_latent_rows(d, N, ch[L]).width) + r16((size_t)in_rows * enc_input_rows(in_K(d), ch[0]).width);
}
size_t net_parts(const lgn_net_desc& d, bool dec, int N) {
  const int* ch = dec ? d.dec_channels : d.enc_channels;
  int rm, rr;
  level_bwd_partial_rows(d.B, N, dec, d.flags, &rm, &rr);
  size_t sum = 0;
  for (int l = 0; l < d.n_levels; ++l) {
    const int H = d.mlp_hidden_mul * 2 * ch[l + 1];
    sum += r16((size_t)rm * 4 * ch[l + 1] * 5 * ch[l]) + r16((size_t)rr * rad_partial_size(ch[l], dec)) +
           r16((size_t)mlp_partial_rows(d.B * (dec ? dec_nodes(d) : N), H) * mlp_psize(ch[l + 1], H, d.mlp_nlin));
  }
  return sum + end_parts(d, dec, N, rm > d.B ? rm : d.B);
}

Work carve(const lgn_net_desc& d, double* base) {
  Work w{};
  Bump b{base};
  const int Nd = dec_nodes(d), Nmax = d.N > Nd ? d.N : Nd;
  const size_t BNe = (size_t)d.B * d.N, BNd = (size_t)d.B * Nd, BN = (size_t)d.B * Nmax;
  const int L = d.n_levels;
  int cmax = 0;
  for (int l = 0; l <= L; ++l) cmax = cmax > d.enc_channels[l] ? cmax : d.enc_channels[l], cmax = cmax > d.dec_channels[l] ? cmax : d.dec_channels[l];
  auto net = [&](NetBuf& n, const int* ch, bool dec) {
    const size_t BN = dec ? BNd : BNe;
    for (int l = 0; l <= L; ++l) {
      n.s[l] = b.take(2 * BN * ch[l]);
      n.v[l] = b.take(8 * BN * ch[l]);
    }
    for (int l = 0; l < L; ++l) {
      n.smix[l] = b.take(2 * BN * ch[l + 1]);
      n.ag0[l] = b.take(4 * BN * ch[l]);
      n.ag1[l] = b.take(16 * BN * ch[l]);
      const size_t hs = l + 1 < L && BN <= mlp_save_max_rows()
                            ? mlp_saved_doubles((int)BN, d.mlp_hidden_mul * 2 * ch[l + 1], d.mlp_nlin) : 0;
      n.hsave[l] = hs ? b.take(hs) : nullptr;
    }
  };
  net(w.enc, d.enc_channels, false);
  net(w.dec, d.dec_channels, true);
  const int Ts = d.tau_s, Tv = d.tau_v, PB = pool_blocks(d.latent_pool);
  w.lat_s = b.take((size_t)2 * d.B * PB * Ts);
  w.lat_v = b.take((size_t)2 * d.B * PB * Tv * 4);
  w.g_lat_v = b.take((size_t)2 * d.B * PB * Tv * 4);
  w.pdec = b.take(8 * BN);
  for (int q = 0; q < 2; ++q) {
    w.gs[q] = b.take(2 * BN * cmax);
    w.gv[q] = b.take(8 * BN * cmax);
  }
  w.gsmix = b.take(2 * BN * cmax);
  w.g_ag = b.take(20 * BN * cmax);
  {
    const size_t z0 = b.off;
    w.zeros_s = b.take(2 * BN * cmax);
    w.g_p = b.take(8 * BN);
    w.g_lat_s = b.take((size_t)2 * d.B * PB * d.tau_s);
    w.tail_cnt = b.take(8);
    w.zero_doubles = b.off - z0;
  }
  w.idx = reinterpret_cast<int*>(b.take(((size_t)d.B * 2 * (Ts + Tv) * 2 + 1) / 2 + 8));
  for (int dec = 0; dec < 2; ++dec)
    for (int l = 0; l < L; ++l) w.tot[dec][l] = b.take(rad_partial_size((dec ? d.dec_channels : d.enc_channels)[l], dec != 0) + 16);
  const size_t psum = net_parts(d, false, d.N) + net_parts(d, true, Nd);
  w.parts = b.take(psum);
  w.parts_size = psum;
  w.total = b.off;
  return w;
}

#define HIPOK(e) do { hipError_t e_ = (e); if (e_ != hipSuccess) { set_error("%s: %s", #e, hipGetErrorString(e_)); return (int)e_; } } while (0)
#define DQ_NEW(var, n) double* var = nullptr; DQ_TAKE(var, n)
#define DQ_TAKE(lhs, n)                                                                                           \
  lhs = dq.take(n);                                                                                             \
  LGN_CHECK_ARG((lhs) != nullptr, "partial-row workspace overflow: %zu + %zu doubles > capacity %zu (carve / take mismatch)", \
                dq.off, (size_t)(n), dq.cap)
#define LGN_TRY(expr)            \
  do {                           \
    int rc_ = (expr);            \
    if (rc_ != 0) return rc_;    \
  } while (0)

struct InputStage {
  const double *w0, *w1;
  double* z1 = nullptr;
  size_t z1n = 0;
  double* z2 = nullptr;
  size_t z2n = 0;
};
struct LossStage {
  const double *wo1, *target;
  double scale;
  int method;
  double jscale;
  double *recon, *loss_part, *g_v, *wpart;
};

MlpArgs<double> level_mlp_args(const lgn_net_desc& d, bool dec, int l, const double* P, const int64_t* off) {
  const Slots S{d.n_levels, d.mlp_nlin};
  const int CO = (dec ? d.dec_channels : d.enc_channels)[l + 1];
  MlpArgs<double> m{};
  m.M = d.B * d.N; m.C = CO; m.H = d.mlp_hidden_mul * 2 * CO; m.nlin = d.mlp_nlin; m.act = d.activation; m.flags = d.flags;
  for (int q = 0; q < d.mlp_nlin; ++q) { m.w[q] = P + off[S.mlp(dec, l, 2 * q)]; m.b[q] = P + off[S.mlp(dec, l, 2 * q + 1)]; }
  return m;
}

int levels_fwd(const lgn_net_desc& d, bool dec, const int* ch, const double* P, const int64_t* off, NetBuf& n, const double* pos,
               const uint8_t* mask, hipStream_t st, const InputStage* in0 = nullptr, const LossStage* loss = nullptr, bool eval = false,
               bool last_scalars = true) {
  const Slots S{d.n_levels, d.mlp_nlin};
  for (int l = 0; l < d.n_levels; ++l) {
    auto p = [&](int slot) { return P + off[slot]; };
    LevelArgs<double> a{d.B, d.N, ch[l], ch[l + 1], n.s[l], n.v[l], pos, mask,
                        p(S.rad(dec, l, 0)), p(S.rad(dec, l, 1)), p(S.rad(dec, l, 2)), p(S.rad(dec, l, 3)), p(S.rad(dec, l, 4)),
                        p(S.rad(dec, l, 5)), p(S.rad(dec, l, 6)), p(S.mix(dec, l, 0)), p(S.mix(dec, l, 1)),
                        n.ag0[l], n.ag1[l], n.smix[l], n.v[l + 1]};
    if (l == 0 && !dec && in0) {
      a.in_w0 = in0->w0; a.in_w1 = in0->w1; a.in_s = n.s[0]; a.in_v = n.v[0];
      a.z1 = in0->z1; a.z1n = in0->z1n; a.z2 = in0->z2; a.z2n = in0->z2n;
    }
    if (l + 1 == d.n_levels && dec && loss) {
      a.loss_wo1 = loss->wo1; a.loss_target = loss->target; a.loss_scale = loss->scale; a.loss_real = loss->method;
      a.loss_jscale = loss->jscale; a.loss_recon = loss->recon;
      a.loss_part = loss->loss_part; a.loss_gv = loss->g_v; a.loss_wpart = loss->wpart;
    }
    a.flags = d.flags;
    LGN_TRY(eval ? level_fwd_eval(a, dec, st) : level_fwd_dispatch<double>(a, dec, st));
    if (l + 1 == d.n_levels && (!last_scalars || (eval && dec))) break;
    MlpArgs<double> m = level_mlp_args(d, dec, l, P, off);
    m.s_in = n.smix[l]; m.s_out = n.s[l + 1];
    m.h_saved = n.hsave[l]; m.h_rows = mlp_saved_rows(m.M);
    LGN_TRY(mlp_dispatch<double>(m, false, st));
  }
  return 0;
}

int levels_bwd(const lgn_net_desc& d, bool dec, const int* ch, const double* P, double* G, const int64_t* off, const NetBuf& n,
               const double* pos, const uint8_t* mask, Work& w, Deferred& dq, RadFinJob& fin, int& cur, bool has_s_grad,
               hipStream_t st, bool* in0_done = nullptr) {
  const Slots S{d.n_levels, d.mlp_nlin};
  const int BN = d.B * d.N;
  for (int l = d.n_levels - 1; l >= 0; --l) {
    auto p = [&](int slot) { return P + off[slot]; };
    auto g = [&](int slot) { return G + off[slot]; };
    const int C = ch[l], CO = ch[l + 1];
    const double* g_smix = w.zeros_s;
    if (has_s_grad) {
      MlpArgs<double> m = level_mlp_args(d, dec, l, P, off);
      m.s_in = n.smix[l]; m.g_out = w.gs[cur]; m.g_in = w.gsmix;
      m.h_saved = n.hsave[l];
      m.h_rows = mlp_saved_rows(BN);
      m.psize = mlp_psize(CO, m.H, m.nlin);
      DQ_TAKE(m.part, (size_t)mlp_partial_rows(BN, m.H) * m.psize);
      LGN_TRY(mlp_dispatch<double>(m, true, st));
      dq.add(m.part, mlp_partial_rows(BN, m.H), m.psize, 0, m.psize, g(S.mlp(dec, l, 0)));
      g_smix = w.gsmix;
    }
    int rm, rr;
    level_bwd_partial_rows(d.B, d.N, dec, d.flags, &rm, &rr);
    const int nmix = 4 * CO * 5 * C, nrad = rad_partial_size(C, dec);
    DQ_NEW(part_mix, (size_t)rm * nmix);
    DQ_NEW(part_rad, (size_t)rr * nrad);
    const int nxt = cur ^ 1;
    LevelBwdArgs<double> a{d.B, d.N, C, CO, n.s[l], n.v[l], pos, mask,
                           p(S.rad(dec, l, 0)), p(S.rad(dec, l, 1)), p(S.rad(dec, l, 2)), p(S.rad(dec, l, 3)), p(S.rad(dec, l, 4)),
                           p(S.rad(dec, l, 5)), p(S.rad(dec, l, 6)), p(S.mix(dec, l, 0)), p(S.mix(dec, l, 1)), n.ag0[l], n.ag1[l],
                           g_smix, w.gv[cur], w.g_ag, w.gs[nxt], w.gv[nxt], dec ? w.g_p : nullptr, part_mix, part_rad};
    const bool carry_in0 = !dec && l == 0 && in0_done && level_bwd_carries_input(d.N, d.flags);
    const RowLayout rin = enc_input_rows(1, C);
    if (carry_in0) { DQ_TAKE(a.part_in0, (size_t)rm * rin.width); }
    a.flags = d.flags;
    LGN_TRY(level_bwd_dispatch<double>(a, dec, st));
    if (carry_in0) {
      rin.add(dq, a.part_in0, rm, G, off);
      *in0_done = true;
    }
    dq.add(part_mix, rm, nmix, 0, nmix / 2, g(S.mix(dec, l, 0)));
    dq.add(part_mix, rm, nmix, nmix / 2, nmix / 2, g(S.mix(dec, l, 1)));
    if (dec) {
      dq.add(part_rad, rr, nrad, 0, C, g(S.rad(dec, l, 4)));
      dq.add(part_rad, rr, nrad, C, C, g(S.rad(dec, l, 6)));
    } else {
      double* tot = w.tot[0][l];
      dq.add(part_rad, rr, nrad, 0, nrad, tot);
      fin.it[fin.n++] = RadFinJob::Item{tot, C, p(S.rad(dec, l, 0)), p(S.rad(dec, l, 1)), p(S.rad(dec, l, 2)), p(S.rad(dec, l, 3)),
                                        p(S.rad(dec, l, 5)), g(S.rad(dec, l, 0)), g(S.rad(dec, l, 1)), g(S.rad(dec, l, 2)),
                                        g(S.rad(dec, l, 3)), g(S.rad(dec, l, 4)), g(S.rad(dec, l, 5)), g(S.rad(dec, l, 6))};
    }
    cur = nxt;
    has_s_grad = true;
  }
  return 0;
}

int check_desc(const lgn_net_desc* d) {
  LGN_CHECK_ARG(d, "step: null descriptor");
  LGN_CHECK_ARG(d->B > 0 && d->N > 0, "step: empty batch (B=%d N=%d)", d->B, d->N);
  LGN_CHECK_ARG(d->n_levels >= 1 && d->n_levels <= 4, "step: n_levels=%d unsupported (1..4)", d->n_levels);
  LGN_CHECK_ARG(d->mlp_nlin >= 4 && d->mlp_nlin <= 7, "step: mlp_depth must be 3 .. 6 (4 .. 7 Linear layers), got %d layers", d->mlp_nlin);
  LGN_CHECK_ARG(d->tau_s >= 1 && d->tau_v >= 1 && d->tau_v_in >= 0, "step: latent multiplicities must be positive");
  LGN_CHECK_ARG(d->n_in_scalars >= 0 && d->n_in_scalars <= 8, "step: n_in_scalars=%d unsupported (0..8)", d->n_in_scalars);
  LGN_CHECK_ARG(pool_valid(d->latent_pool), "step: latent_pool=%d is not an LGN_POOL(...) code", d->latent_pool);
  for (int l = 0; l <= d->n_levels; ++l)
    LGN_CHECK_ARG(d->enc_channels[l] >= 1 && d->enc_channels[l] <= 8 && d->dec_channels[l] >= 1 && d->dec_channels[l] <= 8,
                  "step: channel counts must be in 1..8");
  LGN_CHECK_ARG(d->get_real >= LGN_REAL_SUM && d->get_real <= LGN_REAL_NORM, "step: get_real=%d is not an LGN_REAL_* code", d->get_real);
  LGN_CHECK_ARG(d->jet_loss_scale >= 0.0, "step: jet_loss_scale=%g must be >= 0", d->jet_loss_scale);
  LGN_CHECK_ARG(d->dec_N >= 0, "step: dec_N=%d must be >= 0", d->dec_N);
  if (d->dec_N > 0) {
    const size_t need = decoder_end_lds_bytes(d->dec_N, d->dec_channels[0], dec_tin(*d), d->dec_channels[d->n_levels]);
    LGN_CHECK_ARG(need <= LGN_LDS_LIMIT, "step: dec_N=%d: the decoder end stages need %zu B of LDS (> %d)", d->dec_N, need, LGN_LDS_LIMIT);
  }
  return 0;
}

int plan_assign_loss(const lgn_net_desc* d, const lgn_loss_desc* loss, int* assignment, int* status, AssignLoss& al, const AssignLoss** out) {
  *out = nullptr;
  if (!loss || loss->kind == LGN_LOSS_CHAMFER) return 0;
  if (int rc = check_desc(d)) return rc;
  al = AssignLoss{loss->kind, loss->abs_coord, loss->polar_coord, loss->scale, assignment, status};
  const int Nd = dec_nodes(*d), CL = d->dec_channels[d->n_levels];
  if (int rc = check_assign_loss(al, Nd)) return rc;
  LGN_CHECK_ARG(d->jet_loss_scale == 0.0, "step: jet_loss_scale=%g with loss kind %d: the jet-feature term is a Chamfer option "
                "(--chamfer-jet-features)", d->jet_loss_scale, loss->kind);
  const size_t need = assign_loss_lds_bytes(Nd, CL);
  LGN_CHECK_ARG(need <= LGN_LDS_LIMIT, "step: the assignment-loss stage at N=%d needs %zu B of LDS (> %d)", Nd, need, LGN_LDS_LIMIT);
  *out = &al;
  return 0;
}

}

}


namespace lgn {
namespace {
struct ZeroJob { double* p[3]; size_t n[3]; };
__global__ __launch_bounds__(BLOCK) void zero_ranges_kernel(ZeroJob job) {
  const size_t stride = (size_t)gridDim.x * BLOCK;
#pragma unroll
  for (int q = 0; q < 3; ++q)
    for (size_t i = (size_t)blockIdx.x * BLOCK + threadIdx.x; i < job.n[q]; i += stride) job.p[q][i] = 0.0;
}
int zero_ranges(double* a, size_t na, double* b, size_t nb, double* c, size_t nc, hipStream_t st) {
  const ZeroJob job{{a, b, c}, {a ? na : 0, b ? nb : 0, c ? nc : 0}};
  const size_t most = std::max(job.n[0], std::max(job.n[1], job.n[2]));
  if (!most) return 0;
  const int blocks = (int)std::min<size_t>((most + BLOCK - 1) / BLOCK, 1024);
  hipLaunchKernelGGL(zero_ranges_kernel, dim3(blocks), dim3(BLOCK), 0, st, job);
  LGN_CHECK_LAUNCH();
  return 0;
}
int zero_grads_and_block(double* grads, size_t n, double* zeros, size_t nz, hipStream_t st) {
// ... 731 lines not shown
  dq.cap = w.parts_size;
  RadFinJob fin{};
  int cur = 0;
  {
    const RowLayout ro = dec_output_rows(*d, cd[L]);
    DQ_NEW(part, (size_t)B * ro.width);
    LGN_TRY(dec_output_bwd(B, N, cd[L], a.n.v[L], params + off[S.out0(true) + 1], g_recon, w.gv[cur], part, st));
    ro.add(dq, part, B, grads, off);
  }
  LGN_TRY(levels_bwd(*d, true, cd, params, grads, off, a.n, a.pdec, nullptr, w, dq, fin, cur, false, st));
  {
    const RowLayout ri = dec_input_rows(cd[0], N, Tin);
    DQ_NEW(part, (size_t)B * ri.width);
    LGN_TRY(dec_input_bwd(B, N, cd[0], Tin, lat_v, params + off[1], params + off[3], a.pdec, w.g_p, w.gs[cur], w.gv[cur], g_lat_v, part, st));
    ri.add(dq, part, B, grads, off);
  }
  LGN_CHECK_ARG(dq.off <= dq.cap, "decoder_bwd: partial-row workspace overflow (%zu > %zu)", dq.off, dq.cap);
  return finish_reductions(dq, fin, grads, n_params, nullptr, d->flags, st);
}

}

extern "C" {

int lgn_step_param_slots(const lgn_net_desc* d, int decoder) {
  if (check_desc(d)) return -1;
  return Slots{d->n_levels, d->mlp_nlin}.count(decoder != 0);
}

long long lgn_encoder_end_lds_bytes(int N, int C0, int K, int CL, int Ts, int Tv, int pool) {
  return pool_valid(pool) ? (long long)encoder_end_lds_bytes(N, C0, K < 1 ? 1 : K, CL, Ts, Tv, pool) : -1;
}
long long lgn_decoder_end_lds_bytes(int N, int C0, int Tin, int CL) { return (long long)decoder_end_lds_bytes(N, C0, Tin, CL); }
long long lgn_junction_lds_bytes(int N, int CL, int Ts, int Tv, int pool, int C0) {
  return pool_valid(pool) ? (long long)junction_lds_bytes(N, CL, Ts, Tv, pool, C0) : -1;
}

long long lgn_step_workspace_doubles(const lgn_net_desc* d) {
  if (check_desc(d) || check_latent_match(*d)) return -1;
  if (is_generic(*d, false) || is_generic(*d, true)) {
    if (check_generic(*d, false) || check_generic(*d, true)) return -1;
    return (long long)carve_gen_step(*d, nullptr).total;
  }
  return (long long)carve(*d, nullptr).total;
}

}
static int step_fwd_bwd(const lgn_net_desc* dp, const double* params, double* grads, long long n_params, const int64_t* enc_off,
                        const int64_t* dec_off, const double* p4, const double* target, const uint8_t* mask, const double* in_scalars,
                        double* workspace, long long workspace_doubles, double* recon, double* loss_part, void* stream,
                        const StepTailArgs* tail, const AssignLoss* al = nullptr) {
  if (int rc = check_desc(dp)) return rc;
  const lgn_net_desc& d = *dp;
  LGN_CHECK_ARG(params && grads && enc_off && dec_off && p4 && target && mask && workspace && recon && loss_part && n_params > 0,
                "step_fwd_bwd: null pointer");
  LGN_CHECK_ARG(d.n_in_scalars <= 1 || in_scalars, "step_fwd_bwd: %d input scalars per node, but in_scalars is NULL", d.n_in_scalars);
  if (int rc = check_latent_match(d)) return rc;
  hipStream_t st = (hipStream_t)stream;
  const bool split = step_is_split(d);
  if (is_generic(d, false) || is_generic(d, true)) {
    LGN_CHECK_ARG(!split, "step_fwd_bwd: table-driven networks take the mass as the only input scalar and one node count "
                  "for both networks (n_in_scalars=%d, N=%d, dec_N=%d): use the per-network calls", d.n_in_scalars, d.N, d.dec_N);
    return gen_step_fwd_bwd(d, params, grads, n_params, enc_off, dec_off, p4, target, mask, workspace, workspace_doubles, recon,
                            loss_part, st, tail, al);
  }
  Work w = carve(d, workspace);
  LGN_CHECK_ARG((long long)w.total <= workspace_doubles, "step: workspace holds %lld doubles, this configuration needs %zu",
                workspace_doubles, w.total);
  if (int rc = check_mlp_contiguous(d, false, enc_off)) return rc;
  if (int rc = check_mlp_contiguous(d, true, dec_off)) return rc;
  lgn_net_desc dd = d;
  dd.N = dec_nodes(d);
  const Slots S{d.n_levels, d.mlp_nlin};
  const int L = d.n_levels, B = d.B, Ne = d.N, Nd = dd.N, Ts = d.tau_s, Tv = d.tau_v, K = in_K(d), Tin = dec_tin(d);
  const int* ce = d.enc_channels;
  const int* cd = d.dec_channels;
  const double* wl0 = params + enc_off[S.out0(false)];
  const double* wl1 = params + enc_off[S.out0(false) + 1];
  Deferred dq;
  dq.parts = w.parts;
  dq.cap = w.parts_size;
  RadFinJob fin{};

  if (split) {
    LGN_TRY(zero_ranges(grads, (size_t)n_params, w.zero0(), w.zero_doubles, nullptr, 0, st));
    LGN_TRY(enc_input_fwd(B, Ne, ce[0], K, p4, in_scalars, params + enc_off[0], params + enc_off[1], w.enc.s[0], w.enc.v[0], st));
    LGN_TRY(levels_fwd(d, false, ce, params, enc_off, w.enc, p4, mask, st, nullptr, nullptr, false, false));
    LGN_TRY(enc_latent_fwd(B, Ne, ce[L], Ts, Tv, d.latent_pool, nullptr, w.enc.v[L], wl0, wl1, w.lat_s, w.lat_v, w.idx, st));
    LGN_TRY(dec_input_fwd(B, Nd, cd[0], Tin, w.lat_v, params + dec_off[1], params + dec_off[2], params + dec_off[3], w.pdec, w.dec.s[0],
                          w.dec.v[0], st));
  } else {
    const InputStage in0{params + enc_off[0], params + enc_off[1], grads, (size_t)n_params, w.zeros_s, w.zero_doubles};
    LGN_TRY(levels_fwd(d, false, ce, params, enc_off, w.enc, p4, mask, st, &in0, nullptr, false, false));
    LGN_TRY(junction_fwd(B, Ne, ce[L], Ts, Tv, d.latent_pool, nullptr, w.enc.v[L], wl0, wl1, w.lat_s, w.lat_v, w.idx, cd[0],
                         params + dec_off[1], params + dec_off[2], params + dec_off[3], w.pdec, w.dec.s[0], w.dec.v[0], st));
  }
  int cur = 0;
  {
    const RowLayout ro = dec_output_rows(d, cd[L]);
    DQ_NEW(part, (size_t)B * ro.width);
    const LossStage ls{params + dec_off[S.out0(true) + 1], target, 1.0, d.get_real, d.jet_loss_scale, recon, loss_part, w.gv[cur], part};
    const bool rides = !al && level_fwd_carries_loss(Nd, d.flags);
    LGN_TRY(levels_fwd(dd, true, cd, params, dec_off, w.dec, w.pdec, nullptr, st, nullptr, rides ? &ls : nullptr, false,
                       false));
    if (al)
      LGN_TRY(dec_output_assign_loss(B, Nd, cd[L], w.dec.v[L], ls.wo1, target, ls.method, *al, recon, loss_part, w.gv[cur], part, st));
    else if (!rides)
      LGN_TRY(dec_output_loss(B, Nd, cd[L], w.dec.v[L], ls.wo1, target, 1.0, ls.method, ls.jscale, recon, loss_part, w.gv[cur], part, st));
    ro.add(dq, part, B, grads, dec_off);
  }

  LGN_TRY(levels_bwd(dd, true, cd, params, grads, dec_off, w.dec, w.pdec, nullptr, w, dq, fin, cur, false, st));
  {
    const RowLayout ri = dec_input_rows(cd[0], Nd, Tin), rl = enc_latent_rows(d, Ne, ce[L]);
    DQ_NEW(part, (size_t)B * ri.width);
    DQ_NEW(parte, (size_t)B * rl.width);
    const int rd = cur, wr = cur ^ 1;
    cur = wr;
    if (split) {
      LGN_TRY(dec_input_bwd(B, Nd, cd[0], Tin, w.lat_v, params + dec_off[1], params + dec_off[3], w.pdec, w.g_p, w.gs[rd], w.gv[rd],
                            w.g_lat_v, part, st));
      LGN_TRY(enc_latent_bwd(B, Ne, ce[L], Ts, Tv, d.latent_pool, nullptr, w.enc.v[L], wl0, wl1, w.g_lat_s, w.g_lat_v, w.idx, w.gs[wr],
                             w.gv[wr], parte, st));
    } else {
      LGN_TRY(junction_bwd(B, Ne, cd[0], Tin, w.lat_v, params + dec_off[1], params + dec_off[3], w.pdec, w.g_p, w.gs[rd], w.gv[rd], w.g_lat_v,
                           part, ce[L], Ts, Tv, d.latent_pool, nullptr, w.enc.v[L], wl0, wl1, w.g_lat_s, w.idx, w.gs[wr], w.gv[wr], parte, st));
    }
    ri.add(dq, part, B, grads, dec_off);
    rl.add(dq, parte, B, grads, enc_off);
  }
  bool in0_done = false;
  LGN_TRY(levels_bwd(d, false, ce, params, grads, enc_off, w.enc, p4, mask, w, dq, fin, cur, false, st,
                     split ? nullptr : &in0_done));
  if (!in0_done) {
    const RowLayout ri = enc_input_rows(K, ce[0]);
    DQ_NEW(part, (size_t)B * ri.width);
    LGN_TRY(enc_input_bwd(B, Ne, ce[0], K, p4, split ? in_scalars : nullptr, w.gs[cur], w.gv[cur], part, st));
    ri.add(dq, part, B, grads, enc_off);
  }
  return end_step(dq, fin, grads, n_params, w.tail_cnt, d.flags, tail, st);
}
extern "C" {

int lgn_step_fwd_bwd_f64(const lgn_net_desc* d, const double* params, double* grads, long long n_params, const int64_t* enc_off,
                         const int64_t* dec_off, const double* p4, const double* target, const uint8_t* mask, const double* in_scalars,
                         double* workspace, long long workspace_doubles, double* recon, double* loss_part, const lgn_loss_desc* loss,
                         int* assignment, int* status, void* stream) {
  AssignLoss al;
  const AssignLoss* alp;
  if (int rc = plan_assign_loss(d, loss, assignment, status, al, &alp)) return rc;
  return step_fwd_bwd(d, params, grads, n_params, enc_off, dec_off, p4, target, mask, in_scalars, workspace, workspace_doubles, recon,
                      loss_part, stream, nullptr, alp);
}

int lgn_step_train_f64(const lgn_net_desc* d, double* params, double* grads, long long n_params, const int64_t* enc_off,
                       const int64_t* dec_off, const double* p4, const double* target, const uint8_t* mask, const double* in_scalars,
                       double* workspace, long long workspace_doubles, double* recon, double* loss_part, int n_loss, double l1_lambda,
                       double* adam_m, double* adam_v, long long* step_dev, double lr, double beta1, double beta2, double eps,
                       int do_adam, double* loss_out, const lgn_loss_desc* loss, int* assignment, int* status, void* stream) {
  AssignLoss al;
  const AssignLoss* alp;
  if (int rc = plan_assign_loss(d, loss, assignment, status, al, &alp)) return rc;
  LGN_CHECK_ARG(loss_out && n_loss > 0, "step_train: null pointer");
  LGN_CHECK_ARG(!do_adam || (adam_m && adam_v && step_dev), "step_train: Adam state missing");
  const StepTailArgs tail{params, grads, (long)n_params, adam_m, adam_v, reinterpret_cast<long*>(step_dev), l1_lambda, lr, beta1, beta2,
                          eps, do_adam, loss_part, n_loss, loss_out, 0, nullptr};
  return step_fwd_bwd(d, params, grads, n_params, enc_off, dec_off, p4, target, mask, in_scalars, workspace, workspace_doubles, recon,
                      loss_part, stream, &tail, alp);
}

int lgn_step_finalize_f64(double* params, double* grads, long long n_params, const double* loss_part, int n_loss, double l1_lambda,
                          double* adam_m, double* adam_v, long long* step_dev, double lr, double beta1, double beta2, double eps,
                          int do_adam, double* loss_out, void* stream) {
  LGN_CHECK_ARG(params && grads && loss_part && loss_out && n_params > 0 && n_loss > 0, "step_finalize: null pointer");
  LGN_CHECK_ARG(!do_adam || (adam_m && adam_v && step_dev), "step_finalize: Adam state missing");
  hipStream_t st = (hipStream_t)stream;
  LGN_TRY(finalize_step(params, grads, (long)n_params, loss_part, n_loss, l1_lambda, adam_m, adam_v, reinterpret_cast<long*>(step_dev),
                        lr, beta1, beta2, eps, do_adam, loss_out, st));
  return 0;
}

}

namespace lgn {
namespace {
int optim_tail(const lgn_optim_desc* o, double* params, double* grads, long long n_params, double* state_m, double* state_v,
               long long* step_dev, int do_step, const double* loss_part, int n_loss, double* loss_out, StepTailArgs& t) {
  LGN_CHECK_ARG(o, "optimiser descriptor: null pointer");
  LGN_CHECK_ARG(o->kind == LGN_OPT_ADAM || o->kind == LGN_OPT_RMSPROP, "optimiser descriptor: kind %d is neither LGN_OPT_ADAM nor "
                "LGN_OPT_RMSPROP", o->kind);
  LGN_CHECK_ARG(!do_step || (state_m && state_v && step_dev), "optimiser state missing");
  LGN_CHECK_ARG(o->l2_lambda >= 0.0 && o->eps >= 0.0, "optimiser descriptor: negative l2_lambda or eps");
  LGN_CHECK_ARG(o->kind != LGN_OPT_RMSPROP || (o->alpha >= 0.0 && o->alpha <= 1.0 && o->momentum >= 0.0),
                "optimiser descriptor: RMSprop takes 0 <= alpha <= 1 and momentum >= 0");
  t = StepTailArgs{params, grads, (long)n_params, state_m, state_v, reinterpret_cast<long*>(step_dev), o->l1_lambda, o->lr, o->beta1,
                   o->beta2, o->eps, do_step, loss_part, n_loss, loss_out, 0, nullptr};
  t.opt_form = 1;
  t.kind = o->kind;
  t.l2 = o->l2_lambda;
  t.alpha = o->alpha;
  t.mu = o->momentum;
  return 0;
}
}
}

extern "C" {

int lgn_step_train_opt_f64(const lgn_net_desc* d, double* params, double* grads, long long n_params, const int64_t* enc_off,
                           const int64_t* dec_off, const double* p4, const double* target, const uint8_t* mask, const double* in_scalars,
                           double* workspace, long long workspace_doubles, double* recon, double* loss_part, int n_loss,
                           const lgn_optim_desc* opt, double* state_m, double* state_v, long long* step_dev, int do_step,
                           double* loss_out, const lgn_loss_desc* loss, int* assignment, int* status, void* stream) {
  lgn::AssignLoss al;
  const lgn::AssignLoss* alp;
  if (int rc = lgn::plan_assign_loss(d, loss, assignment, status, al, &alp)) return rc;
  LGN_CHECK_ARG(loss_out && n_loss > 0, "step_train_opt: null pointer");
  lgn::StepTailArgs tail{};
  if (int rc = lgn::optim_tail(opt, params, grads, n_params, state_m, state_v, step_dev, do_step, loss_part, n_loss, loss_out, tail))
    return rc;
  return step_fwd_bwd(d, params, grads, n_params, enc_off, dec_off, p4, target, mask, in_scalars, workspace, workspace_doubles,
                           recon, loss_part, stream, &tail, alp);
}

int lgn_step_finalize_opt_f64(double* params, double* grads, long long n_params, const double* loss_part, int n_loss,
                              const lgn_optim_desc* opt, double* state_m, double* state_v, long long* step_dev, int do_step,
                              double* loss_out, void* stream) {
  LGN_CHECK_ARG(params && grads && loss_part && loss_out && n_params > 0 && n_loss > 0, "step_finalize_opt: null pointer");
  lgn::StepTailArgs tail{};
  if (int rc = lgn::optim_tail(opt, params, grads, n_params, state_m, state_v, step_dev, do_step, loss_part, n_loss, loss_out, tail))
    return rc;
  return lgn::finalize_step_opt(tail, (hipStream_t)stream);
}

}

namespace lgn {
namespace {

struct EvalWork {
  NetBuf enc, dec;
  double *lat_s, *lat_v, *pdec;
  int* idx;
  size_t total;
};

EvalWork carve_eval(const lgn_net_desc& d, double* base) {
  EvalWork w{};
  Bump b{base};
  const int L = d.n_levels, Nd = dec_nodes(d);
  const size_t BNe = (size_t)d.B * d.N, BNd = (size_t)d.B * Nd;
  size_t smix = 0;
  auto net = [&](NetBuf& n, const int* ch, size_t BN) {
    int cmax = 0;
    for (int l = 0; l <= L; ++l) cmax = cmax > ch[l] ? cmax : ch[l];
    double *s[2], *v[2];
    for (int q = 0; q < 2; ++q) {
      s[q] = b.take(2 * BN * cmax);
      v[q] = b.take(8 * BN * cmax);
    }
    for (int l = 0; l <= L; ++l) {
      n.s[l] = s[l & 1];
      n.v[l] = v[l & 1];
    }
    smix = std::max(smix, 2 * BN * cmax);
  };
  net(w.enc, d.enc_channels, BNe);
  net(w.dec, d.dec_channels, BNd);
  double* sm = b.take(smix);
  for (int l = 0; l < L; ++l) w.enc.smix[l] = w.dec.smix[l] = sm;
  const int PB = pool_blocks(d.latent_pool);
  w.lat_s = b.take((size_t)2 * d.B * PB * d.tau_s);
  w.lat_v = b.take((size_t)2 * d.B * PB * d.tau_v * 4);
  w.pdec = b.take(8 * BNd);
  w.idx = reinterpret_cast<int*>(b.take(((size_t)d.B * 2 * (d.tau_s + d.tau_v) * 2 + 1) / 2 + 8));
  w.total = b.off;
  return w;
}

struct GenEval {
  GenAct ea, da;
  double *lat_s, *lat_v;
  size_t total;
};
GenEval carve_gen_eval(const lgn_net_desc& d, double* base) {
  GenEval g{};
  auto at = [&](size_t off) { return base ? base + off : nullptr; };
  size_t off = 0;
  g.ea = carve_gen_act(d, false, at(off)); off += (g.ea.total + 15) & ~size_t(15);
  g.da = carve_gen_act(d, true, at(off)); off += (g.da.total + 15) & ~size_t(15);
  const int P = pool_blocks(d.latent_pool);
  g.lat_s = at(off); off += ((size_t)2 * d.B * P * d.tau_s + 15) & ~size_t(15);
  g.lat_v = at(off); off += ((size_t)2 * d.B * P * d.tau_v * 4 + 15) & ~size_t(15);
  g.total = off;
  return g;
}

long long eval_workspace(const lgn_net_desc& d) {
  if (is_generic(d, false) || is_generic(d, true)) {
    if (check_generic(d, false) || check_generic(d, true)) return -1;
    return (long long)carve_gen_eval(d, nullptr).total;
  }
  return (long long)carve_eval(d, nullptr).total;
}

int step_eval(const lgn_net_desc* dp, const double* params, const int64_t* enc_off, const int64_t* dec_off, const double* p4,
              const double* target, const uint8_t* mask, const double* in_scalars, double* workspace, long long workspace_doubles,
              double* recon_real, double* lat_s_out, double* lat_v_out, double* loss_part, double* loss_out, hipStream_t st,
              const AssignLoss* al) {
  if (int rc = check_desc(dp)) return rc;
  const lgn_net_desc& d = *dp;
  LGN_CHECK_ARG(params && enc_off && dec_off && p4 && target && mask && workspace && recon_real && loss_part && loss_out,
                "step_eval: null pointer");
  LGN_CHECK_ARG(d.n_in_scalars <= 1 || in_scalars, "step_eval: %d input scalars per node, but in_scalars is NULL", d.n_in_scalars);
  LGN_CHECK_ARG(!lat_s_out == !lat_v_out, "step_eval: give both latent outputs or neither");
  if (int rc = check_latent_match(d)) return rc;
  const long long need = eval_workspace(d);
  if (need < 0) return -1;
  LGN_CHECK_ARG(need <= workspace_doubles, "step_eval: workspace holds %lld doubles, this configuration needs %lld", workspace_doubles, need);
  if (int rc = check_mlp_contiguous(d, false, enc_off)) return rc;
  if (int rc = check_mlp_contiguous(d, true, dec_off)) return rc;
  const Slots S{d.n_levels, d.mlp_nlin};
  const int L = d.n_levels, B = d.B, Ne = d.N, Nd = dec_nodes(d), Ts = d.tau_s, Tv = d.tau_v, Tin = dec_tin(d);
  const int* ce = d.enc_channels;
  const int* cd = d.dec_channels;
  const double* wl0 = params + enc_off[S.out0(false)];
  const double* wl1 = params + enc_off[S.out0(false) + 1];
  const double* wo1 = params + dec_off[S.out0(true) + 1];

  if (is_generic(d, false) || is_generic(d, true)) {
    LGN_CHECK_ARG(is_generic(d, false) && is_generic(d, true), "step_eval: encoder and decoder must both be table-driven (or both fused)");
    LGN_CHECK_ARG(!step_is_split(d), "step_eval: table-driven networks take the mass as the only input scalar and one node count for "
                  "both networks (n_in_scalars=%d, N=%d, dec_N=%d)", d.n_in_scalars, d.N, d.dec_N);
    GenEval g = carve_gen_eval(d, workspace);
    double* ls = lat_s_out ? lat_s_out : g.lat_s;
    double* lv = lat_v_out ? lat_v_out : g.lat_v;
    LGN_TRY(gen_encoder_fwd(d, params, enc_off, p4, mask, g.ea, ls, lv, st, nullptr, false));
    LGN_TRY(junction_fwd(B, Ne, ce[L], Ts, Tv, d.latent_pool, g.ea.sL, g.ea.vL, wl0, wl1, ls, lv, g.ea.idx, cd[0], params + dec_off[1],
                         params + dec_off[2], params + dec_off[3], g.da.pdec, g.da.s0, g.da.v0, st));
    LGN_TRY(gen_decoder_fwd(d, params, dec_off, lv, g.da, st, false));
    if (al) LGN_TRY(dec_output_assign_eval(B, Ne, cd[L], g.da.vL, wo1, target, d.get_real, *al, recon_real, loss_part, st));
    else LGN_TRY(dec_output_eval(B, Ne, cd[L], g.da.vL, wo1, target, d.get_real, d.jet_loss_scale, recon_real, loss_part, st));
    return eval_loss_sum(B, Ne, mask, loss_part, loss_out, st);
  }

  EvalWork w = carve_eval(d, workspace);
  double* ls = lat_s_out ? lat_s_out : w.lat_s;
  double* lv = lat_v_out ? lat_v_out : w.lat_v;
  lgn_net_desc dd = d;
  dd.N = Nd;
  const LossStage loss{wo1, target, 1.0, d.get_real, d.jet_loss_scale, recon_real, loss_part, nullptr, nullptr};
  const bool rides = !al && level_fwd_carries_loss(Nd, d.flags);
  const bool keep_s = lat_s_out != nullptr;
  const double* sL = keep_s ? w.enc.s[L] : nullptr;
  if (step_is_split(d)) {
    LGN_TRY(enc_input_fwd(B, Ne, ce[0], in_K(d), p4, in_scalars, params + enc_off[0], params + enc_off[1], w.enc.s[0], w.enc.v[0], st));
    LGN_TRY(levels_fwd(d, false, ce, params, enc_off, w.enc, p4, mask, st, nullptr, nullptr, true, keep_s));
    LGN_TRY(enc_latent_fwd(B, Ne, ce[L], Ts, Tv, d.latent_pool, sL, w.enc.v[L], wl0, wl1, ls, lv, w.idx, st));
    LGN_TRY(dec_input_fwd(B, Nd, cd[0], Tin, lv, params + dec_off[1], params + dec_off[2], params + dec_off[3], w.pdec, w.dec.s[0],
                          w.dec.v[0], st));
  } else {
    const InputStage in0{params + enc_off[0], params + enc_off[1]};
    LGN_TRY(levels_fwd(d, false, ce, params, enc_off, w.enc, p4, mask, st, &in0, nullptr, true, keep_s));
    LGN_TRY(junction_fwd(B, Ne, ce[L], Ts, Tv, d.latent_pool, sL, w.enc.v[L], wl0, wl1, ls, lv, w.idx, cd[0],
                         params + dec_off[1], params + dec_off[2], params + dec_off[3], w.pdec, w.dec.s[0], w.dec.v[0], st));
  }
  LGN_TRY(levels_fwd(dd, true, cd, params, dec_off, w.dec, w.pdec, nullptr, st, nullptr, rides ? &loss : nullptr, true));
  if (al) LGN_TRY(dec_output_assign_eval(B, Nd, cd[L], w.dec.v[L], wo1, target, d.get_real, *al, recon_real, loss_part, st));
  else if (!rides) LGN_TRY(dec_output_eval(B, Nd, cd[L], w.dec.v[L], wo1, target, d.get_real, d.jet_loss_scale, recon_real, loss_part, st));
  return eval_loss_sum(B, Ne, mask, loss_part, loss_out, st);
}

}
}

extern "C" {

long long lgn_eval_workspace_doubles(const lgn_net_desc* d) {
  if (check_desc(d)) return -1;
  return eval_workspace(*d);
}

int lgn_step_eval_f64(const lgn_net_desc* d, const double* params, const int64_t* enc_off, const int64_t* dec_off,
                      const double* p4_scaled, const double* p4_target, const uint8_t* mask, const double* in_scalars,
                      double* workspace, long long workspace_doubles, double* recon_real, double* lat_s, double* lat_v,
                      double* loss_part, double* loss_out, const lgn_loss_desc* loss, int* assignment, int* status, void* stream) {
  AssignLoss al;
  const AssignLoss* alp;
  if (int rc = plan_assign_loss(d, loss, assignment, status, al, &alp)) return rc;
  return step_eval(d, params, enc_off, dec_off, p4_scaled, p4_target, mask, in_scalars, workspace, workspace_doubles, recon_real, lat_s,
                   lat_v, loss_part, loss_out, (hipStream_t)stream, alp);
}

}
```

### lgn-autoencoder_amd/lgn/_native.py

```python
from __future__ import annotations

import ctypes as C
import os
from typing import Optional, Sequence

import torch

_HERE = os.path.dirname(os.path.abspath(__file__))
LIB_PATH = os.environ.get("LGN_AMD_LIB") or os.path.join(_HERE, "_lib", "liblgn_amd.so")
ABI_VERSION = 19
FINALIZE_SCRATCH = 2048
FINALIZE_OPT_SCRATCH = 4096

_lib: Optional[C.CDLL] = None

_vp, _i, _ip = C.c_void_p, C.c_int, C.POINTER(C.c_int)

_SIGNATURES = {
    "lgn_level_fwd_f64": [_i] * 5 + [_vp] * 18,
    "lgn_level_bwd_partial_rows": [_i, _i, _i, _ip, _ip],
    "lgn_level_rad_partial_len": [_i, _i],
    "lgn_level_jet_split": [_i, _i],
    "lgn_cg_product_fwd_f64": [_i] * 8 + [_vp] * 7,
    "lgn_cg_product_bwd_f64": [_i] * 8 + [_vp] * 9,
    "lgn_level_bwd_f64": [_i] * 5 + [_vp] * 24,
    "lgn_reduce_partials_f64": [_vp, _i, _i, _vp, _i, _vp],
    "lgn_radial_finalize_f64": [_vp, _i] + [_vp] * 13,
    "lgn_cgmlp_fwd_f64": [_i] * 5 + [_vp] * 5,
    "lgn_cgmlp_partial_rows": [_i, _i],
    "lgn_cgmlp_bwd_f64": [_i] * 5 + [_vp] * 6 + [_i, _vp],
    "lgn_mixreps_fwd_f64": [_i] * 4 + [_vp] * 4,
    "lgn_chamfer_f64": [_i] * 3 + [_vp] * 2 + [_i] + [_vp] * 4,
    "lgn_mixreps_partial_rows": [_i],
    "lgn_mixreps_bwd_f64": [_i] * 4 + [_vp] * 6,
}


class LocalTables(C.Structure):
    _fields_ = [("n_rows", C.c_int), ("n_out", C.c_int), ("n_w", C.c_int), ("n_terms", C.c_int), ("n_u", C.c_int),
                ("n_x", C.c_int), ("n_units", C.c_int), ("static_kind", C.c_int)] + [
        (name, C.c_void_p) for name in ("row_ptr", "t_type", "t_a", "t_b", "t_coef", "out_dim", "out_nblk", "out_row0", "out_q0",
                                        "out_w0", "u_ptr", "u_row", "u_coef", "x_ptr", "x_row", "x_other", "x_coef")] + [("h_out_w0", C.c_int * 8)]


_tp = C.POINTER(LocalTables)


_POOL_OPS = {"min": 0, "max": 1, "mean": 2, "average": 2}


def pool_code(map_to_latent: str):
    m = map_to_latent.lower()
    if m == "mix":
        return 1 | (3 << 4)
    if "&" in m and "+" in m:
        return None
    avg = "+" in m
    ops = m.split("+") if avg else m.split("&")
    if not 1 <= len(ops) <= 4 or any(o not in _POOL_OPS for o in ops):
        return None
    code = len(ops) | (int(avg) << 3)
    for i, o in enumerate(ops):
        code |= _POOL_OPS[o] << (4 + 2 * i)
    return code


def end_stages_fit(encoder=None, decoder=None, junction: bool = False) -> bool:
    L = lib()
    need = 0
    if encoder is not None:
        code = pool_code(encoder.map_to_latent)
        if code is None:
            return False
        n = encoder.num_input_particles
        ch = encoder.num_channels
        ts, tv = encoder.tau_latent[(0, 0)], encoder.tau_latent[(1, 1)]
        need = max(need, L.lgn_encoder_end_lds_bytes(n, ch[0], max(1, encoder.tau_input_scalars), ch[-1], ts, tv, code))
        if junction and decoder is not None:
            need = max(need, L.lgn_junction_lds_bytes(n, ch[-1], ts, tv, code, decoder.num_channels[0]))
    if decoder is not None:
        ch = decoder.num_channels
        need = max(need, L.lgn_decoder_end_lds_bytes(decoder.num_output_particles, ch[0], decoder.tau_latent_vectors, ch[-1]))
    return 0 <= need <= LDS_LIMIT


def pool_blocks(code: int) -> int:
    if code == 0:
        return 2
    return 1 if (code >> 3) & 1 else code & 7


class NetDesc(C.Structure):
    _fields_ = [("B", C.c_int), ("N", C.c_int), ("n_levels", C.c_int), ("enc_channels", C.c_int * 5),
                ("dec_channels", C.c_int * 5), ("tau_s", C.c_int), ("tau_v", C.c_int), ("mlp_hidden_mul", C.c_int),
                ("mlp_nlin", C.c_int), ("tau_v_in", C.c_int),
                ("enc_tables", _tp * 4), ("dec_tables", _tp * 4),
                ("enc_Q", C.c_int * 5), ("enc_qs", C.c_int * 5), ("enc_qv", C.c_int * 5),
                ("dec_Q", C.c_int * 5), ("dec_qs", C.c_int * 5), ("dec_qv", C.c_int * 5), ("flags", C.c_int),
                ("activation", C.c_int), ("n_in_scalars", C.c_int), ("latent_pool", C.c_int), ("dec_N", C.c_int),
                ("get_real", C.c_int), ("jet_loss_scale", C.c_double)]

    def __init__(self, *a, **kw):
        super().__init__(*a, **kw)
        self.flags = net_flags()


NET_NO_STATIC = 1
_NET_FLAG_ENV = {"LGN_AMD_NO_STATIC": 1, "LGN_AMD_DEC_PAIRWISE": 2, "LGN_AMD_LEVEL_V2": 4, "LGN_AMD_MLP_V1": 8,
                 "LGN_AMD_MOMENTS_V1": 16, "LGN_AMD_BWD_ORDERED": 64, "LGN_AMD_SPLIT_TAIL": 128, "LGN_AMD_DEC_UNFUSED": 256, "LGN_AMD_MOMENTS_SPLIT": 512,
                 "LGN_AMD_MLP_BWD1": 1024}
ACTIVATIONS = {"leakyrelu": 0, "relu": 1, "elu": 2, "sigmoid": 3, "logsigmoid": 4, "atan": 5}


def activation_id(name: str) -> int:
    try:
        return ACTIVATIONS[name.lower()]
    except KeyError:
        raise ValueError(f"Activation function {name} not implemented!") from None


def net_flags() -> int:
    return sum(bit for name, bit in _NET_FLAG_ENV.items() if os.environ.get(name, "") == "1")


class LossDesc(C.Structure):
    _fields_ = [("kind", C.c_int), ("abs_coord", C.c_int), ("polar_coord", C.c_int), ("scale", C.c_double)]


class OptimDesc(C.Structure):
    _fields_ = [("kind", C.c_int), ("l1_lambda", C.c_double), ("l2_lambda", C.c_double), ("lr", C.c_double), ("eps", C.c_double),
                ("beta1", C.c_double), ("beta2", C.c_double), ("alpha", C.c_double), ("momentum", C.c_double)]


OPT_ADAM, OPT_RMSPROP = 0, 1
LOSS_CHAMFER, LOSS_MSE, LOSS_HUNGARIAN = 0, 1, 2
ASSIGN_NMAX = 192
_dp = C.POINTER(NetDesc)
_lp = C.POINTER(LossDesc)
_op = C.POINTER(OptimDesc)
_ll = C.c_longlong
_d = C.c_double
_SIGNATURES.update({
    "lgn_moments_fwd_f64": [_i] * 5 + [_vp] * 12,
    "lgn_moments_bwd_f64": [_i] * 5 + [_vp] * 16,
    "lgn_local_fwd_f64": [_i] * 5 + [_tp] + [_vp] * 5,
    "lgn_local_partial_rows": [_i],
    "lgn_local_fwd_static_f64": [_i] * 4 + [_vp] * 3 + [_ip] + [_vp] * 3 + [_i, _vp],
    "lgn_local_bwd_static_f64": [_i] * 4 + [_vp] * 3 + [_ip] + [_vp] * 8,
    "lgn_local_bwd_f64": [_i] * 5 + [_tp] + [_vp] * 8,
    "lgn_step_param_slots": [_dp, _i],
    "lgn_step_fwd_bwd_f64": [_dp, _vp, _vp, _ll, _vp, _vp, _vp, _vp, _vp, _vp, _vp, _ll, _vp, _vp, _lp, _vp, _vp, _vp],
    "lgn_encoder_fwd_f64": [_dp, _vp, _vp, _vp, _vp, _vp, _vp, _ll, _vp, _vp, _vp],
    "lgn_encoder_bwd_f64": [_dp, _vp, _vp, _ll, _vp, _vp, _vp, _vp, _vp, _ll, _vp, _vp, _vp, _ll, _vp],
    "lgn_decoder_fwd_f64": [_dp, _vp, _vp, _vp, _vp, _ll, _vp, _vp],
    "lgn_decoder_bwd_f64": [_dp, _vp, _vp, _ll, _vp, _vp, _vp, _ll, _vp, _vp, _vp, _ll, _vp],
    "lgn_step_finalize_f64": [_vp, _vp, _ll, _vp, _i, _d, _vp, _vp, _vp, _d, _d, _d, _d, _i, _vp, _vp],
    "lgn_step_train_f64": [_dp, _vp, _vp, _ll, _vp, _vp, _vp, _vp, _vp, _vp, _vp, _ll, _vp, _vp, _i, _d, _vp, _vp, _vp, _d, _d, _d, _d, _i,
                           _vp, _lp, _vp, _vp, _vp],
    "lgn_step_finalize_opt_f64": [_vp, _vp, _ll, _vp, _i, _op, _vp, _vp, _vp, _i, _vp, _vp],
    "lgn_step_train_opt_f64": [_dp, _vp, _vp, _ll, _vp, _vp, _vp, _vp, _vp, _vp, _vp, _ll, _vp, _vp, _i, _op, _vp, _vp, _vp, _i, _vp, _lp,
                               _vp, _vp, _vp],
    "lgn_step_eval_f64": [_dp, _vp, _vp, _vp, _vp, _vp, _vp, _vp, _vp, _ll, _vp, _vp, _vp, _vp, _vp, _lp, _vp, _vp, _vp],
    "lgn_anomaly_scores_f64": [_vp] * 4 + [_i] * 3 + [_vp] * 4,
    "lgn_linear_sum_assignment_f64": [_vp, _i, _i, _vp, _vp, _vp],
    "lgn_hungarian_mse_f64": [_i, _i, _vp, _vp, _i, _i, _i, _d] + [_vp] * 5,
    "lgn_recon_analysis_f64": [_vp, _vp] + [_i] * 4 + [_vp] * 11,
    "lgn_match_rel_err_f64": [_vp] * 6 + [_i, _i] + [_vp] * 5,
    "lgn_histogram_f64": [_vp, _ll, _i, _i, _vp, _ip, _i, _vp, _vp, _vp, _vp, _i, _vp],
    "lgn_stage_batch_f64": [_vp] * 3 + [_i] * 4 + [_d, _i, _i] + [_vp] * 6,
    "lgn_denormalize_f64": [_vp] * 3 + [_i, _i] + [_vp] * 3,
    "lgn_stage_gather_f64": [_vp] * 3 + [_ll, _vp, _ll, _vp] + [_i] * 3 + [_d, _i, _i] + [_vp] * 7,
    "lgn_epoch_collect_f64": [_vp] * 3 + [_ll, _i, _i, C.POINTER(_vp), C.POINTER(_vp), _ip, _vp],
    "lgn_epoch_reset": [_vp] * 4,
    "lgn_roc_auc_f64": [_vp, _ll, _i, _i] + [_vp] * 9 + [_ll, _vp],
    "lgn_emd_f64": [_vp, _vp, _i, _i, _i, _d] + [_vp] * 6 + [_ll, _vp],
    "lgn_emd_relative_f64": [_vp, _vp, _i, _i, _vp, _vp, _vp, _ll, _vp],
    "lgn_emd_debug_max_augmentations": [_ip, _i],
    "lgn_column_stats_f64": [_vp, _ll, _i, _i, _vp, _i, _d, _i] + [_vp] * 5 + [_ll, _vp],
    "lgn_hist_fwhm_f64": [_vp, _i, _vp, _i, _ip, _i, _vp, _vp],
    "lgn_jet_images_f64": [_vp, _vp, _i, _i, _i, _i, _d, _i, _vp, _vp, _vp, _ll, _vp],
    "lgn_transform_jets_f64": [_vp] * 4 + [_i] * 4 + [_vp] * 3,
    "lgn_rep_deviation_f64": [_i] * 3 + [C.POINTER(_vp)] * 3 + [_ip] * 3 + [_vp] * 3 + [_ll, _vp],
})
EPOCH_MAX_COLLECT, EPOCH_BAD_INDEX = 4, 1
NORM_NONE, NORM_COMPONENT_MAX, NORM_OVERALL_MAX, NORM_JET_E = 0, 1, 2, 3


_LL_SIGNATURES = {
    "lgn_step_workspace_doubles": [_dp],
    "lgn_eval_workspace_doubles": [_dp],
    "lgn_net_workspace_doubles": [_dp, _i, _i],
    "lgn_moments_scratch_doubles": [_i, _i, _i, _i],
    "lgn_local_static_packed_doubles": [_i, _i, _i],
    "lgn_encoder_end_lds_bytes": [_i] * 7,
    "lgn_decoder_end_lds_bytes": [_i] * 4,
    "lgn_junction_lds_bytes": [_i] * 6,
    "lgn_assign_loss_lds_bytes": [_i, _i],
    "lgn_roc_workspace_bytes": [_ll, _i],
    "lgn_emd_workspace_bytes": [_i, _i],
    "lgn_emd_lds_bytes": [_i],
    "lgn_column_stats_workspace_bytes": [_ll, _i],
    "lgn_jet_images_workspace_bytes": [_i, _i],
    "lgn_rep_deviation_workspace_bytes": [_i, _i, _i, _ip, _ip, _ip],
}
ROC_TILE, ROC_MAX_COLS = 2048, 65535
# ... 292 lines not shown
```

Before: 1.066 million.

## Skip masked particle groups in encoder sweeps and sort jets by occupancy

Adds a default-on path in the encoder level forward and backward kernels that skips 4-particle groups with no unmasked particles. It builds a per-jet active-group bitmask with a ballot and accounts for the skipped groups through closed-form channel sums, so the gradients for masked pairs stay correct. A new single-block kernel sorts jets by active-group count and interleaves heavy and light jets across CUs to balance the load of the 2D grid. The change adds an extra kernel launch per step, extra reductions and LDS use, and numerical-equivalence risk in the closed-form correction.

Measured after the change: 1.046 million. 0.981x the previous value.

```diff
diff --git a/include/lgn_amd.h b/include/lgn_amd.h
--- a/include/lgn_amd.h
+++ b/include/lgn_amd.h
@@ -23,6 +23,7 @@
 int lgn_level_bwd_partial_rows(int B, int N, int decoder, int* rows_mix, int* rows_rad);
 int lgn_level_rad_partial_len(int C, int decoder);
 int lgn_level_jet_split(int B, int N);
+int lgn_jet_order(int B, int N, int ncu, const uint8_t* mask, int* order, void* stream);
 
 int lgn_level_bwd_f64(int B, int N, int C, int CO, int decoder,
                       const double* s_in, const double* v_in, const double* p, const uint8_t* mask,
@@ -149,6 +150,8 @@
 #define LGN_NET_DEC_UNFUSED 256
 #define LGN_NET_MOMENTS_SPLIT 512
 #define LGN_NET_MLP_BWD1 1024
+#define LGN_NET_ENC_FULL_SWEEP 2048
+#define LGN_NET_JET_IDENTITY 4096
 #define LGN_NET_SPLIT_TAIL 128
 
 #define LGN_LDS_LIMIT (160 * 1024)
diff --git a/lgn-autoencoder_amd/csrc/api.hip b/lgn-autoencoder_amd/csrc/api.hip
--- a/lgn-autoencoder_amd/csrc/api.hip
+++ b/lgn-autoencoder_amd/csrc/api.hip
@@ -13,6 +13,10 @@
   LevelArgs<double> a{B, N, C, CO, s_in, v_in, p, mask, ra, rb, rc, w0, b0, w1, b1, wm0, wm1, ag0, ag1, s_out, v_out};
   a.flags = level_flags_from_env();
   return level_fwd_dispatch<double>(a, decoder, (hipStream_t)stream);
+}
+
+int lgn_jet_order(int B, int N, int ncu, const uint8_t* mask, int* order, void* stream) {
+  return jet_order_table(B, N, ncu, mask, order, (hipStream_t)stream);
 }
 
 int lgn_level_bwd_partial_rows(int B, int N, int decoder, int* rows_mix, int* rows_rad) {
diff --git a/lgn-autoencoder_amd/csrc/api_common.cpp b/lgn-autoencoder_amd/csrc/api_common.cpp
--- a/lgn-autoencoder_amd/csrc/api_common.cpp
+++ b/lgn-autoencoder_amd/csrc/api_common.cpp
@@ -16,11 +16,13 @@
   auto on = [](const char* name) { const char* e = getenv(name); return e && e[0] == '1'; };
   return (on("LGN_AMD_DEC_PAIRWISE") ? LVL_DEC_PAIRWISE : 0) | (on("LGN_AMD_LEVEL_V2") ? LVL_LEVEL_V2 : 0) |
          (on("LGN_AMD_MOMENTS_V1") ? LVL_MOMENTS_V1 : 0) | (on("LGN_AMD_MLP_V1") ? LVL_MLP_V1 : 0) | (on("LGN_AMD_BWD_ORDERED") ? LVL_BWD_ORDERED : 0) |
-         (on("LGN_AMD_MOMENTS_SPLIT") ? LVL_MOMENTS_SPLIT : 0) | (on("LGN_AMD_MLP_BWD1") ? LVL_MLP_BWD1 : 0);
+         (on("LGN_AMD_MOMENTS_SPLIT") ? LVL_MOMENTS_SPLIT : 0) | (on("LGN_AMD_MLP_BWD1") ? LVL_MLP_BWD1 : 0) |
+         (on("LGN_AMD_ENC_FULL_SWEEP") ? LVL_ENC_FULL_SWEEP : 0);
 }
 static_assert(LVL_DEC_PAIRWISE == LGN_NET_DEC_PAIRWISE && LVL_LEVEL_V2 == LGN_NET_LEVEL_V2 && LVL_MOMENTS_V1 == LGN_NET_MOMENTS_V1 &&
                   LVL_MLP_V1 == LGN_NET_MLP_V1 && LVL_MLP_BWD1 == LGN_NET_MLP_BWD1 &&
-                  LVL_BWD_ORDERED == LGN_NET_BWD_ORDERED && LVL_MOMENTS_SPLIT == LGN_NET_MOMENTS_SPLIT, "LVL_* and LGN_NET_* are the same bits");
+                  LVL_BWD_ORDERED == LGN_NET_BWD_ORDERED && LVL_MOMENTS_SPLIT == LGN_NET_MOMENTS_SPLIT &&
+                  LVL_ENC_FULL_SWEEP == LGN_NET_ENC_FULL_SWEEP && LVL_JET_IDENTITY == LGN_NET_JET_IDENTITY, "LVL_* and LGN_NET_* are the same bits");
 }
 
 extern "C" {
diff --git a/lgn-autoencoder_amd/csrc/level.hpp b/lgn-autoencoder_amd/csrc/level.hpp
--- a/lgn-autoencoder_amd/csrc/level.hpp
+++ b/lgn-autoencoder_amd/csrc/level.hpp
@@ -10,6 +10,8 @@
 constexpr int LVL_MLP_BWD1 = 1024;
 constexpr int LVL_MOMENTS_SPLIT = 512;
 constexpr int LVL_BWD_ORDERED = 64;
+constexpr int LVL_ENC_FULL_SWEEP = 2048;
+constexpr int LVL_JET_IDENTITY = 4096;
 int level_flags_from_env();
 
 template <typename T>
@@ -43,6 +45,7 @@
   T* loss_gv = nullptr;
   T* loss_wpart = nullptr;
   int flags = 0;
+  const int* jet_order = nullptr;
 };
 
 template <typename T>
@@ -63,6 +66,7 @@
   T* part_rad;
   T* part_in0 = nullptr;
   int flags = 0;
+  const int* jet_order = nullptr;
 };
 
 __host__ __device__ constexpr int node_stride(int C) { return 10 * C + 4; }
diff --git a/lgn-autoencoder_amd/csrc/level_bwd3.hip b/lgn-autoencoder_amd/csrc/level_bwd3.hip
--- a/lgn-autoencoder_amd/csrc/level_bwd3.hip
+++ b/lgn-autoencoder_amd/csrc/level_bwd3.hip
@@ -73,7 +73,7 @@
   using G = GA3<C>;
   constexpr int NG = F::NG, NS = F::NS, PS = F::PS, K = 5 * C;
   const int N = a.N, B = a.B, CO = a.CO;
-  const int b = blockIdx.x, tid = threadIdx.x, lane = tid & 63, wave = tid >> 6;
+  const int b = a.jet_order ? a.jet_order[blockIdx.x] : blockIdx.x, tid = threadIdx.x, lane = tid & 63, wave = tid >> 6;
   const int ngroups = (N + 3) >> 2, gper = (ngroups + (int)gridDim.y - 1) / (int)gridDim.y;
   const int glo = min(ngroups, (int)blockIdx.y * gper), ghi = min(ngroups, glo + gper);
   const int nlo = min(N, 4 * glo), nhi = min(N, 4 * ghi);
@@ -508,6 +508,156 @@
   __syncthreads();
   STAMP(5);
 
+  const int gcount = ghi - glo;
+  const int rs = (!SYM && !DEC && NWV == 4 && gcount >= 1 && gcount <= 2) ? NWV / gcount : 1;
+  const bool ts = !DEC && gridDim.y == 1 && rs == 1 && !(a.flags & LVL_ENC_FULL_SWEEP);
+  unsigned act = 0, allg = 0;
+  if (ts) {
+    const unsigned long long bal = __ballot(lane < N && mk[lane < N ? lane : 0] != 0);
+    for (int g = 0; g < ngroups; ++g) act |= ((bal >> (4 * g)) & 0xF) ? 1u << g : 0u;
+    act = __builtin_amdgcn_readfirstlane(act);
+    allg = (1u << ngroups) - 1;
+  }
+  const bool cform = ts && act != allg;
+  __shared__ double dbcf[32];
+  if constexpr (!DEC) {
+    if (cform) {
+      constexpr int SMS = 52;
+      double* cfs = tr;
+      for (int c = wave; c < C; c += NWV) {
+        double t0[16], t1[16], t2[12], t3[8];
+        const bool in = lane < N;
+        const int n = in ? lane : 0;
+        const double* ni = nd + n * NS + c * 10;
+        const double* pn = pj + n * 4;
+        const double* gi = ga + n * G::SIZE;
+        const double h = rsqrt2<double>();
+        const cx<double> pc[4] = {{pn[0], 0.0}, {pn[1] * h, -pn[2] * h}, {pn[3], 0.0}, {-pn[1] * h, -pn[2] * h}};
+        cx<double> v[4];
+#pragma unroll
+        for (int m = 0; m < 4; ++m) v[m] = {ni[2 + m], ni[6 + m]};
+        const cx<double> sn = {ni[0], ni[1]};
+        t0[0] = sn.r;  t0[1] = sn.i;
+#pragma unroll
+        for (int m = 0; m < 4; ++m) {
+          t0[2 + 2 * m] = v[m].r;  t0[3 + 2 * m] = v[m].i;
+          const cx<double> sp = cmul(sn, pc[m]);
+          if (m < 3) { t0[10 + 2 * m] = sp.r;  t0[11 + 2 * m] = sp.i; }
+          else { t1[0] = sp.r;  t1[1] = sp.i; }
+        }
+        const cx<double> vp = bil2(v, pc);
+        t1[2] = vp.r;  t1[3] = vp.i;
+        const cx<double> g3 = {0.5 * gi[G::A3 + 2 * c], 0.5 * gi[G::A3 + 2 * c + 1]};
+        t1[4] = gi[G::A4 + 2 * c];  t1[5] = gi[G::A4 + 2 * c + 1];
+        t1[6] = g3.r;  t1[7] = g3.i;
+        cx<double> gp2 = {0, 0};
+#pragma unroll
+        for (int m = 0; m < 4; ++m) {
+          const cx<double> g1 = {gi[G::A1 + (c * 4 + m) * 2], gi[G::A1 + (c * 4 + m) * 2 + 1]};
+          const cx<double> g2 = {gi[G::A2 + (c * 4 + m) * 2], gi[G::A2 + (c * 4 + m) * 2 + 1]};
+          t1[8 + 2 * m] = g1.r;  t1[9 + 2 * m] = g1.i;
+          t2[2 * m] = g2.r;  t2[2 * m + 1] = g2.i;
+          cfmac(gp2, g2, pc[m]);
+          const cx<double> gp3 = cmulc(g3, pc[m]);
+          if (m == 0) { t2[10] = gp3.r;  t2[11] = gp3.i; }
+          else { t3[2 * m - 2] = gp3.r;  t3[2 * m - 1] = gp3.i; }
+        }
+        t2[8] = gp2.r;  t2[9] = gp2.i;
+        t3[6] = t3[7] = 0.0;
+#pragma unroll
+        for (int pass = 1; pass >= 0; --pass) {
+          if (pass == 1 ? !in : (((act >> (n >> 2)) & 1) != 0)) {
+#pragma unroll
+            for (int k = 0; k < 16; ++k) t0[k] = t1[k] = 0.0;
+#pragma unroll
+            for (int k = 0; k < 12; ++k) t2[k] = 0.0;
+#pragma unroll
+            for (int k = 0; k < 8; ++k) t3[k] = 0.0;
+          }
+          double* q = cfs + (pass * C + c) * SMS;
+          wave_sum_store<16>(t0, q, lane);
+          wave_sum_store<16>(t1, q + 16, lane);
+          wave_sum_store<12>(t2, q + 32, lane);
+          wave_sum_store<8>(t3, q + 44, lane);
+        }
+      }
+      __syncthreads();
+      for (int e = tid; e < N * C; e += BLK) {
+        const int n = e / C, c = e - n * C;
+        const double* q = cfs + ((((act >> (n >> 2)) & 1) ? 0 : C) + c) * SMS;
+        const double* pn = pj + n * 4;
+        double* gdn = gd + e * 10;
+        const cx<double> R0 = {a.b0[2 * c], a.b0[2 * c + 1]}, R1 = {a.b1[2 * c], a.b1[2 * c + 1]};
+        const cx<double> e0 = {R0.r - R0.i, R0.r + R0.i};
+        const double h = rsqrt2<double>();
+        const cx<double> pc[4] = {{pn[0], 0.0}, {pn[1] * h, -pn[2] * h}, {pn[3], 0.0}, {-pn[1] * h, -pn[2] * h}};
+        cx<double> pt[4];
+        metric_perm(pc, pt);
+        const cx<double> SG4 = {q[20], q[21]}, SG3 = {q[22], q[23]}, GP2 = {q[40], q[41]};
+        cx<double> GP3[4], GPT3[4];
+#pragma unroll
+        for (int m = 0; m < 4; ++m) GP3[m] = {q[42 + 2 * m], q[43 + 2 * m]};
+        metric_perm(GP3, GPT3);
+        cx<double> u = GP2;
+#pragma unroll
+        for (int m = 0; m < 4; ++m) {
+          const cx<double> t = cmulc(cx<double>{q[32 + 2 * m], q[33 + 2 * m]}, pc[m]);
+          u.r -= t.r;  u.i -= t.i;
+        }
+        cx<double> gs = cmulc(SG4, e0);
+        cfmac(gs, u, R1);
+        gdn[0] += gs.r;
+        gdn[1] += gs.i;
+#pragma unroll
+        for (int m = 0; m < 4; ++m) {
+          cx<double> w = GPT3[m];
+          const cx<double> t = cmulc(SG3, pt[m]);
+          w.r -= t.r;  w.i -= t.i;
+          cx<double> gv = cmulc(cx<double>{q[24 + 2 * m], q[25 + 2 * m]}, e0);
+          cfmac(gv, w, R1);
+          gdn[2 + m] += gv.r;
+          gdn[6 + m] += gv.i;
+        }
+      }
+      if (tid < 2 * C) {
+        const int lin = tid / C, c = tid - lin * C;
+        const double* qm = cfs + c * SMS;
+        const double* qa = cfs + (C + c) * SMS;
+        auto E0 = [&](const double* qg, const double* qf) {
+          cx<double> r = cmulc(cx<double>{qg[20], qg[21]}, cx<double>{qf[0], qf[1]});
+#pragma unroll
+          for (int m = 0; m < 4; ++m) cfmac(r, cx<double>{qg[24 + 2 * m], qg[25 + 2 * m]}, cx<double>{qf[2 + 2 * m], qf[3 + 2 * m]});
+          return r;
+        };
+        auto E1 = [&](const double* qg, const double* qf) {
+          cx<double> VS[4], VSt[4];
+#pragma unroll
+          for (int m = 0; m < 4; ++m) VS[m] = {qf[2 + 2 * m], qf[3 + 2 * m]};
+          metric_perm(VS, VSt);
+          cx<double> r = cmulc(cx<double>{qg[40], qg[41]}, cx<double>{qf[0], qf[1]});
+          cx<double> neg = cmulc(cx<double>{qg[22], qg[23]}, cx<double>{qf[18], qf[19]});
+#pragma unroll
+          for (int m = 0; m < 4; ++m) {
+            cfmac(neg, cx<double>{qg[32 + 2 * m], qg[33 + 2 * m]}, cx<double>{qf[10 + 2 * m], qf[11 + 2 * m]});
+            cfmac(r, cx<double>{qg[42 + 2 * m], qg[43 + 2 * m]}, VSt[m]);
+          }
+          return cx<double>{r.r - neg.r, r.i - neg.i};
+        };
+        if (lin == 0) {
+          const cx<double> x = E0(qa, qm), y = E0(qm, qm), z = E0(qm, qa);
+          const cx<double> ge0 = {(x.r - y.r) + z.r, (x.i - y.i) + z.i};
+          dbcf[2 * c] = ge0.r + ge0.i;
+          dbcf[2 * c + 1] = ge0.i - ge0.r;
+        } else {
+          const cx<double> x = E1(qa, qm), y = E1(qm, qm), z = E1(qm, qa);
+          dbcf[2 * C + 2 * c] = (x.r - y.r) + z.r;
+          dbcf[2 * C + 2 * c + 1] = (x.i - y.i) + z.i;
+        }
+      }
+      __syncthreads();
+    }
+  }
+
   double* trw = tr + wave * (NG + 3) * 16 * TS;
   v4d T[NG][3];
   double dB0[NG], dB1[NG];
@@ -521,17 +671,27 @@
   double in0[NG][4];
 #pragma unroll
   for (int g = 0; g < NG; ++g) in0[g][0] = in0[g][1] = in0[g][2] = in0[g][3] = 0.0;
-  const int gcount = ghi - glo;
-  const int rs = (!SYM && !DEC && NWV == 4 && gcount >= 1 && gcount <= 2) ? NWV / gcount : 1;
   const int rpart = rs > 1 ? wave % rs : 0;
   const int ntl = (N + 3) >> 2, i0lo = rs > 1 ? 4 * (rpart * ntl / rs) : 0, i0hi = rs > 1 ? min(N, 4 * ((rpart + 1) * ntl / rs)) : N;
+  auto nth = [&](unsigned bits, int k) {
+    for (int t = 0; t < k && bits; ++t) bits &= bits - 1;
+    return bits ? (int)__builtin_ctz(bits) : -1;
+  };
+  const int nact = ts ? __builtin_popcount(act) : ngroups;
   for (int u = 0;; ++u) {
     int rg;
     if constexpr (SYM) {
-      const int p = wave + NWV * (u >> 1);
-      if (p >= (ngroups + 1) >> 1) break;
-      rg = (u & 1) ? ngroups - 1 - p : p;
-      if ((u & 1) && rg == p) continue;
+      const int hp = (nact + 1) >> 1, na = hp > wave ? (hp - wave + NWV - 1) / NWV : 0;
+      if (u < 2 * na) {
+        const int p = wave + NWV * (u >> 1);
+        const int ck = (u & 1) ? nact - 1 - p : p;
+        if ((u & 1) && ck == p) continue;
+        rg = ts ? nth(act, ck) : ck;
+      } else {
+        if (!ts) break;
+        rg = nth(allg & ~act, wave + NWV * (u - 2 * na));
+        if (rg < 0) break;
+      }
     } else if (rs > 1) {
       if (u > 0) break;
       rg = glo + wave / rs;
@@ -566,7 +726,13 @@
 #pragma unroll
     for (int m = 0; m < 4; ++m) Gq[m] = {0, 0};
 
-    for (int i0 = i0lo; i0 < i0hi; i0 += 4) {
+    const bool swept = !ts || ((act >> rg) & 1);
+    auto nxt = [&](int i0) {
+      if (!ts) return i0 + 4;
+      const unsigned r = (act >> (i0 >> 2)) >> 1;
+      return r ? i0 + 4 * (1 + (int)__builtin_ctz(r)) : i0hi;
+    };
+    for (int i0 = !ts ? i0lo : (swept ? 4 * (int)__builtin_ctz(act) : i0hi); i0 < i0hi; i0 = nxt(i0)) {
       if (rg == glo && i0 < 32) STAMP(16 + (i0 >> 2) * 4);
       const int kind = SYM ? ((i0 >> 2) < rg ? 2 : ((i0 >> 2) == rg ? 1 : 0)) : 1;
       const int i = i0 + ti;
@@ -970,7 +1136,7 @@
               if (col < 4) part[r * NB + 16 + col] = v;
               else if (col < 8) part[R * NB + r * NB + 16 + (col - 4)] = v;
               else if (col == 8) part[2 * R * NB + r] = v;
-              else if (col == 9) part[2 * R * NB + R + r] = v;
+              else if (col == 9) part[2 * R * NB + R + r] = cform ? v + dbcf[r] : v;
             }
           }
       }
diff --git a/lgn-autoencoder_amd/csrc/level_fwd2.hip b/lgn-autoencoder_amd/csrc/level_fwd2.hip
--- a/lgn-autoencoder_amd/csrc/level_fwd2.hip
+++ b/lgn-autoencoder_amd/csrc/level_fwd2.hip
@@ -48,7 +48,7 @@
   using F = Fwd2<C, DEC>;
   constexpr int NG = F::NG;
   const int N = a.N, B = a.B, CO = a.CO;
-  const int b = blockIdx.x, tid = threadIdx.x, lane = tid & 63, wave = tid >> 6;
+  const int b = a.jet_order ? a.jet_order[blockIdx.x] : blockIdx.x, tid = threadIdx.x, lane = tid & 63, wave = tid >> 6;
   const int nthr = blockDim.x, nw = nthr >> 6;
 
   extern __shared__ __align__(16) unsigned char smem_raw[];
@@ -57,7 +57,7 @@
   double* wm = pj + N * F::PS;
   double* agl = wm + 4 * CO * 5 * C;
   double* sums = agl + chunk * F::AGS;
-  uint8_t* mk = reinterpret_cast<uint8_t*>(sums + 20 * C);
+  uint8_t* mk = reinterpret_cast<uint8_t*>(sums + 40 * C);
 
   STAMP(0);
   if (!DEC && a.in_w0) {
@@ -208,6 +208,58 @@
 
   const int ngroups = (N + 3) >> 2, gper = (ngroups + (int)gridDim.y - 1) / (int)gridDim.y;
   const int rlo = min(N, 4 * (int)blockIdx.y * gper), rhi = min(N, rlo + 4 * gper);
+  const bool ts = !DEC && !SEP && gridDim.y == 1 && N <= 40 && ngroups > 2 && chunk >= N && !(a.flags & LVL_ENC_FULL_SWEEP);
+  unsigned act = 0, allg = 0;
+  if (ts) {
+    const unsigned long long bal = __ballot(lane < N && mk[lane < N ? lane : 0] != 0);
+    for (int g = 0; g < ngroups; ++g) act |= ((bal >> (4 * g)) & 0xF) ? 1u << g : 0u;
+    act = __builtin_amdgcn_readfirstlane(act);
+    allg = (1u << ngroups) - 1;
+  }
+  const bool cform = ts && act != allg;
+  if constexpr (!DEC && !SEP) {
+    if (cform) {
+      for (int c = wave; c < C; c += nw) {
+        double a0[12], a1[8];
+        const bool in = lane < N;
+        const int n = in ? lane : 0;
+        const double* ni = nd + n * F::NS + c * 10;
+        const double* pn = pj + n * 4;
+        const double h = rsqrt2<double>();
+        const cx<double> pc[4] = {{pn[0], 0.0}, {pn[1] * h, -pn[2] * h}, {pn[3], 0.0}, {-pn[1] * h, -pn[2] * h}};
+        const cx<double> sn = {ni[0], ni[1]};
+        cx<double> v[4];
+#pragma unroll
+        for (int m = 0; m < 4; ++m) v[m] = {ni[2 + m], ni[6 + m]};
+        const cx<double> vp = bil2(v, pc);
+        a0[0] = sn.r;  a0[1] = sn.i;
+#pragma unroll
+        for (int m = 0; m < 4; ++m) {
+          a0[2 + 2 * m] = v[m].r;  a0[3 + 2 * m] = v[m].i;
+          const cx<double> sp = cmul(sn, pc[m]);
+          if (m == 0) { a0[10] = sp.r;  a0[11] = sp.i; }
+          else { a1[2 * m - 2] = sp.r;  a1[2 * m - 1] = sp.i; }
+        }
+        a1[6] = vp.r;  a1[7] = vp.i;
+        if (!in) {
+#pragma unroll
+          for (int k = 0; k < 12; ++k) a0[k] = 0.0;
+#pragma unroll
+          for (int k = 0; k < 8; ++k) a1[k] = 0.0;
+        }
+        wave_sum_store<12>(a0, sums + 20 * C + c * 20, lane);
+        wave_sum_store<8>(a1, sums + 20 * C + c * 20 + 12, lane);
+        if ((act >> (n >> 2)) & 1) {
+#pragma unroll
+          for (int k = 0; k < 12; ++k) a0[k] = 0.0;
+#pragma unroll
+          for (int k = 0; k < 8; ++k) a1[k] = 0.0;
+        }
+        wave_sum_store<12>(a0, sums + c * 20, lane);
+        wave_sum_store<8>(a1, sums + c * 20 + 12, lane);
+      }
+    }
+  }
   auto catmix = [&](int c0, int c1) {
     constexpr int K = 5 * C;
     const int nr = c1 - c0;
@@ -417,18 +469,23 @@
         }
       }
     };
+    auto nxt = [&](int j) {
+      if (!ts) return j + 4;
+      const unsigned r = (act >> (j >> 2)) >> 1;
+      return r ? j + 4 * (1 + __builtin_ctz(r)) : jhi;
+    };
     if (jlo < jhi) {
       Tile ta, tb;
       prep(jlo, ta);
       int j0 = jlo;
       while (true) {
-        if (j0 + 4 < jhi) prep(j0 + 4, tb);
+        const int j1 = nxt(j0);
+        if (j1 < jhi) prep(j1, tb);
         agg(ta);
-        j0 += 4;
-        if (j0 >= jhi) break;
-        if (j0 + 4 < jhi) prep(j0 + 4, ta);
+        if (j1 >= jhi) break;
+        j0 = nxt(j1);
+        if (j0 < jhi) prep(j0, ta);
         agg(tb);
-        j0 += 4;
         if (j0 >= jhi) break;
       }
     }
@@ -466,7 +523,17 @@
     const int rg = (c0 >> 2) + wave / rs;
     if (rg * 4 < c1) row_group(rg, 4 * (rpart * ntl / rs), min(N, 4 * ((rpart + 1) * ntl / rs)), rpart * 4 * ngr);
   } else {
-    for (int rg = (c0 >> 2) + wave; rg * 4 < c1; rg += nw) row_group(rg, 0, N, 0);
+    const int jfirst = ts ? (act ? 4 * __builtin_ctz(act) : N) : 0;
+    for (int k = wave;; k += nw) {
+      int rg = (c0 >> 2) + k;
+      if (ts) {
+        unsigned rem = act;
+        for (int t = 0; t < k && rem; ++t) rem &= rem - 1;
+        if (!rem) break;
+        rg = __builtin_ctz(rem);
+      } else if (rg * 4 >= c1) break;
+      row_group(rg, jfirst, N, 0);
+    }
   }
   if (rs > 1) {
     __syncthreads();
@@ -479,6 +546,42 @@
   }
   }
   __syncthreads();
+  if constexpr (!DEC && !SEP) {
+    if (cform) {
+      for (int e = tid; e < N * C; e += nthr) {
+        const int n = e / C, c = e - n * C;
+        const bool ract = (act >> (n >> 2)) & 1;
+        const double* sm = sums + (ract ? 0 : 20 * C) + c * 20;
+        const double* pn = pj + n * 4;
+        const double h = rsqrt2<double>();
+        const cx<double> pc[4] = {{pn[0], 0.0}, {pn[1] * h, -pn[2] * h}, {pn[3], 0.0}, {-pn[1] * h, -pn[2] * h}};
+        const cx<double> R0 = {a.b0[2 * c], a.b0[2 * c + 1]}, R1 = {a.b1[2 * c], a.b1[2 * c + 1]};
+        const cx<double> e0 = {R0.r - R0.i, R0.r + R0.i};
+        const cx<double> S = {sm[0], sm[1]};
+        cx<double> VS[4];
+#pragma unroll
+        for (int m = 0; m < 4; ++m) VS[m] = {sm[2 + 2 * m], sm[3 + 2 * m]};
+        double* st = agl + n * F::AGS;
+        const cx<double> a4 = cmul(S, e0);
+        cx<double> t = bil2(VS, pc);
+        t.r -= sm[18];  t.i -= sm[19];
+        const cx<double> a3 = cmul(R1, t);
+        auto put = [&](double* d, double v) { *d = ract ? *d + v : v; };
+        put(st + F::A3 + 2 * c, 0.5 * a3.r);  put(st + F::A3 + 2 * c + 1, 0.5 * a3.i);
+        put(st + F::A4 + 2 * c, a4.r);        put(st + F::A4 + 2 * c + 1, a4.i);
+#pragma unroll
+        for (int m = 0; m < 4; ++m) {
+          const cx<double> a1 = cmul(VS[m], e0);
+          cx<double> u = cmul(pc[m], S);
+          u.r -= sm[10 + 2 * m];  u.i -= sm[11 + 2 * m];
+          const cx<double> a2 = cmul(R1, u);
+          put(st + F::A1 + (c * 4 + m) * 2, a1.r);  put(st + F::A1 + (c * 4 + m) * 2 + 1, a1.i);
+          put(st + F::A2 + (c * 4 + m) * 2, a2.r);  put(st + F::A2 + (c * 4 + m) * 2 + 1, a2.i);
+        }
+      }
+      __syncthreads();
+    }
+  }
   STAMP(20);
 
   if constexpr (TRAIN) {
@@ -517,7 +620,7 @@
 template <int C, bool DEC, bool SEP, bool TRAIN>
 static int launch_level_fwd2(const LevelArgs<double>& a, hipStream_t stream) {
   using F = Fwd2<C, DEC>;
-  const size_t fixed = sizeof(double) * (((size_t)a.N * F::NS + 1 & ~size_t(1)) + (size_t)a.N * F::PS + 4 * a.CO * 5 * C + 20 * C) + a.N + 16;
+  const size_t fixed = sizeof(double) * (((size_t)a.N * F::NS + 1 & ~size_t(1)) + (size_t)a.N * F::PS + 4 * a.CO * 5 * C + 40 * C) + a.N + 16;
   const bool wide = a.B <= 320 && a.N >= 64;
   const size_t row = sizeof(double) * F::AGS, budget1 = 160 * 1024, budget2 = wide ? budget1 : 78 * 1024;
   const int full = (a.N + 15) & ~15;
@@ -577,6 +680,84 @@
   return level_fwd_run<true>(a, decoder, stream);
 }
 
+constexpr int JO_MAXB = 4096, JO_MAXKEY = 64, JO_THREADS = 256, JO_STAGE = 24576;
+__global__ __launch_bounds__(JO_THREADS) void jet_order_kernel(int B, int N, int ncu, const uint8_t* __restrict__ mask, int* __restrict__ order) {
+  const int tid = threadIdx.x, lane = tid & 63, wave = tid >> 6;
+  if (!(ncu < B && B <= 2 * ncu && B <= JO_MAXB)) {
+    for (int i = tid; i < B; i += JO_THREADS) order[i] = i;
+    return;
+  }
+  __shared__ uint8_t key[JO_MAXB];
+  __shared__ int seg[(JO_MAXB / 64) * JO_MAXKEY];
+  __shared__ int srt[JO_MAXB];
+  __shared__ __align__(16) uint8_t stage[JO_STAGE];
+  const int ng = (N + 3) >> 2, nseg = (B + 63) >> 6;
+  const size_t bytes = (size_t)B * N;
+  const bool staged = bytes <= JO_STAGE;
+  if (staged) {
+    if ((reinterpret_cast<uintptr_t>(mask) & 3) == 0) {
+      const uint32_t* src = reinterpret_cast<const uint32_t*>(mask);
+      uint32_t* dst = reinterpret_cast<uint32_t*>(stage);
+      for (size_t e = tid; e < bytes / 4; e += JO_THREADS) dst[e] = src[e];
+      for (size_t e = (bytes & ~size_t(3)) + tid; e < bytes; e += JO_THREADS) stage[e] = mask[e];
+    } else {
+      for (size_t e = tid; e < bytes; e += JO_THREADS) stage[e] = mask[e];
+    }
+    __syncthreads();
+  }
+  for (int b = tid; b < B; b += JO_THREADS) {
+    const uint8_t* m = (staged ? stage : mask) + (size_t)b * N;
+    int k = 0;
+    for (int g = 0; g < ng; ++g) {
+      int any = 0;
+      for (int e = 4 * g; e < min(N, 4 * g + 4); ++e) any |= m[e];
+      k += any != 0;
+    }
+    key[b] = (uint8_t)k;
+  }
+  __syncthreads();
+  for (int sg = wave; sg < nseg; sg += JO_THREADS / 64) {
+    const int b = sg * 64 + lane, k = b < B ? key[b] : -1;
+    for (int kk = 0; kk <= ng; ++kk) {
+      const unsigned long long m = __ballot(k == kk);
+      if (lane == 0) seg[sg * JO_MAXKEY + kk] = __popcll(m);
+    }
+  }
+  __syncthreads();
+  if (tid <= ng) {
+    int start = 0;
+    for (int k2 = tid + 1; k2 <= ng; ++k2)
+      for (int sg = 0; sg < nseg; ++sg) start += seg[sg * JO_MAXKEY + k2];
+    for (int sg = 0; sg < nseg; ++sg) {
+      const int c = seg[sg * JO_MAXKEY + tid];
+      seg[sg * JO_MAXKEY + tid] = start;
+      start += c;
+    }
+  }
+  __syncthreads();
+  for (int sg = wave; sg < nseg; sg += JO_THREADS / 64) {
+    const int b = sg * 64 + lane, k = b < B ? key[b] : -1;
+    for (int kk = 0; kk <= ng; ++kk) {
+      const unsigned long long m = __ballot(k == kk);
+      if (k == kk) srt[seg[sg * JO_MAXKEY + kk] + __popcll(m & ((1ull << lane) - 1))] = b;
+    }
+  }
+  __syncthreads();
+  for (int i = tid; i < B; i += JO_THREADS) order[i] = i < ncu ? srt[i] : srt[B - 1 - (i - ncu)];
+}
+
+int jet_order_table(int B, int N, int ncu, const uint8_t* mask, int* order, hipStream_t stream) {
+  LGN_CHECK_ARG(B > 0 && N > 0 && ncu > 0 && mask && order, "jet_order: bad arguments (B=%d N=%d ncu=%d)", B, N, ncu);
+  LGN_CHECK_ARG((N + 3) / 4 < JO_MAXKEY, "jet_order: N=%d unsupported (<= %d)", N, 4 * (JO_MAXKEY - 1));
+  hipLaunchKernelGGL(jet_order_kernel, dim3(1), dim3(JO_THREADS), 0, stream, B, N, ncu, mask, order);
+  LGN_CHECK_LAUNCH();
+  return 0;
+}
+
+bool jet_order_applies(int B, int N, int ncu, int flags) {
+  return N <= 40 && level_jet_split(B, N) == 1 && ncu < B && B <= 2 * ncu && B <= JO_MAXB && !(flags & LVL_JET_IDENTITY);
+}
+
 int level_fwd_eval(const LevelArgs<double>& a, int decoder, hipStream_t stream) { return level_fwd_run<false>(a, decoder, stream); }
 
 }
diff --git a/lgn-autoencoder_amd/csrc/ops.hpp b/lgn-autoencoder_amd/csrc/ops.hpp
--- a/lgn-autoencoder_amd/csrc/ops.hpp
+++ b/lgn-autoencoder_amd/csrc/ops.hpp
@@ -46,6 +46,8 @@
 int step_tail(const std::vector<RedSeg<double>>& segs, const RadFinJob& fin, const StepTailArgs& ta, hipStream_t st);
 void level_bwd_partial_rows(int B, int N, int decoder, int flags, int* rows_mix, int* rows_rad);
 bool level_bwd_carries_input(int N, int flags);
+int jet_order_table(int B, int N, int ncu, const uint8_t* mask, int* order, hipStream_t);
+bool jet_order_applies(int B, int N, int ncu, int flags);
 bool level_fwd_carries_loss(int N, int flags);
 
 constexpr int MLP_MAX_LIN = 8;
diff --git a/lgn-autoencoder_amd/csrc/step.hip b/lgn-autoencoder_amd/csrc/step.hip
--- a/lgn-autoencoder_amd/csrc/step.hip
+++ b/lgn-autoencoder_amd/csrc/step.hip
@@ -24,6 +24,7 @@
 struct NetBuf {
   double *s[5], *v[5], *smix[4], *ag0[4], *ag1[4];
   double* hsave[4];
+  const int* jet_order = nullptr;
 };
 
 struct Work {
@@ -34,6 +35,7 @@
   size_t parts_size;
   double* tot[2][4];
   int* idx;
+  int* jet_order;
   size_t total;
   double* tail_cnt;
   double* zero0() const { return tail_cnt < zeros_s ? tail_cnt : zeros_s; }
@@ -206,6 +208,7 @@
     w.zero_doubles = b.off - z0;
   }
   w.idx = reinterpret_cast<int*>(b.take(((size_t)d.B * 2 * (Ts + Tv) * 2 + 1) / 2 + 8));
+  w.jet_order = reinterpret_cast<int*>(b.take(((size_t)d.B + 1) / 2));
   for (int dec = 0; dec < 2; ++dec)
     for (int l = 0; l < L; ++l) w.tot[dec][l] = b.take(rad_partial_size((dec ? d.dec_channels : d.enc_channels)[l], dec != 0) + 16);
   const size_t psum = net_parts(d, false, d.N) + net_parts(d, true, Nd);
@@ -249,6 +252,26 @@
   m.M = d.B * d.N; m.C = CO; m.H = d.mlp_hidden_mul * 2 * CO; m.nlin = d.mlp_nlin; m.act = d.activation; m.flags = d.flags;
   for (int q = 0; q < d.mlp_nlin; ++q) { m.w[q] = P + off[S.mlp(dec, l, 2 * q)]; m.b[q] = P + off[S.mlp(dec, l, 2 * q + 1)]; }
   return m;
+}
+
+static int device_cus() {
+  static thread_local int dev_of = -1, cus = -1;
+  int dev = 0;
+  if (hipGetDevice(&dev) != hipSuccess) return -1;
+  if (dev != dev_of) {
+    int v = 0;
+    if (hipDeviceGetAttribute(&v, hipDeviceAttributeMultiprocessorCount, dev) != hipSuccess) return -1;
+    dev_of = dev;
+    cus = v;
+  }
+  return cus;
+}
+static int step_jet_order(const lgn_net_desc& d, const uint8_t* mask, int* table, NetBuf& enc, hipStream_t st) {
+  const int ncu = device_cus();
+  if (ncu <= 0 || !jet_order_applies(d.B, d.N, ncu, d.flags)) return 0;
+  LGN_TRY(jet_order_table(d.B, d.N, ncu, mask, table, st));
+  enc.jet_order = table;
+  return 0;
 }
 
 int levels_fwd(const lgn_net_desc& d, bool dec, const int* ch, const double* P, const int64_t* off, NetBuf& n, const double* pos,
@@ -271,6 +294,7 @@
       a.loss_part = loss->loss_part; a.loss_gv = loss->g_v; a.loss_wpart = loss->wpart;
     }
     a.flags = d.flags;
+    a.jet_order = n.jet_order;
     LGN_TRY(eval ? level_fwd_eval(a, dec, st) : level_fwd_dispatch<double>(a, dec, st));
     if (l + 1 == d.n_levels && (!last_scalars || (eval && dec))) break;
     MlpArgs<double> m = level_mlp_args(d, dec, l, P, off);
@@ -316,6 +340,7 @@
     const RowLayout rin = enc_input_rows(1, C);
     if (carry_in0) { DQ_TAKE(a.part_in0, (size_t)rm * rin.width); }
     a.flags = d.flags;
+    a.jet_order = n.jet_order;
     LGN_TRY(level_bwd_dispatch<double>(a, dec, st));
     if (carry_in0) {
       rin.add(dq, a.part_in0, rm, G, off);
@@ -1213,6 +1238,7 @@
   dq.cap = w.parts_size;
   RadFinJob fin{};
 
+  LGN_TRY(step_jet_order(d, mask, w.jet_order, w.enc, st));
   if (split) {
     LGN_TRY(zero_ranges(grads, (size_t)n_params, w.zero0(), w.zero_doubles, nullptr, 0, st));
     LGN_TRY(enc_input_fwd(B, Ne, ce[0], K, p4, in_scalars, params + enc_off[0], params + enc_off[1], w.enc.s[0], w.enc.v[0], st));
@@ -1373,6 +1399,7 @@
   NetBuf enc, dec;
   double *lat_s, *lat_v, *pdec;
   int* idx;
+  int* jet_order;
   size_t total;
 };
 
@@ -1405,6 +1432,7 @@
   w.lat_v = b.take((size_t)2 * d.B * PB * d.tau_v * 4);
   w.pdec = b.take(8 * BNd);
   w.idx = reinterpret_cast<int*>(b.take(((size_t)d.B * 2 * (d.tau_s + d.tau_v) * 2 + 1) / 2 + 8));
+  w.jet_order = reinterpret_cast<int*>(b.take(((size_t)d.B + 1) / 2));
   w.total = b.off;
   return w;
 }
@@ -1484,6 +1512,7 @@
   const bool rides = !al && level_fwd_carries_loss(Nd, d.flags);
   const bool keep_s = lat_s_out != nullptr;
   const double* sL = keep_s ? w.enc.s[L] : nullptr;
+  LGN_TRY(step_jet_order(d, mask, w.jet_order, w.enc, st));
   if (step_is_split(d)) {
     LGN_TRY(enc_input_fwd(B, Ne, ce[0], in_K(d), p4, in_scalars, params + enc_off[0], params + enc_off[1], w.enc.s[0], w.enc.v[0], st));
     LGN_TRY(levels_fwd(d, false, ce, params, enc_off, w.enc, p4, mask, st, nullptr, nullptr, true, keep_s));
diff --git a/lgn-autoencoder_amd/lgn/_native.py b/lgn-autoencoder_amd/lgn/_native.py
--- a/lgn-autoencoder_amd/lgn/_native.py
+++ b/lgn-autoencoder_amd/lgn/_native.py
@@ -21,6 +21,7 @@
     "lgn_level_bwd_partial_rows": [_i, _i, _i, _ip, _ip],
     "lgn_level_rad_partial_len": [_i, _i],
     "lgn_level_jet_split": [_i, _i],
+    "lgn_jet_order": [_i, _i, _i, _vp, _vp, _vp],
     "lgn_cg_product_fwd_f64": [_i] * 8 + [_vp] * 7,
     "lgn_cg_product_bwd_f64": [_i] * 8 + [_vp] * 9,
     "lgn_level_bwd_f64": [_i] * 5 + [_vp] * 24,
@@ -108,7 +109,8 @@
 NET_NO_STATIC = 1
 _NET_FLAG_ENV = {"LGN_AMD_NO_STATIC": 1, "LGN_AMD_DEC_PAIRWISE": 2, "LGN_AMD_LEVEL_V2": 4, "LGN_AMD_MLP_V1": 8,
                  "LGN_AMD_MOMENTS_V1": 16, "LGN_AMD_BWD_ORDERED": 64, "LGN_AMD_SPLIT_TAIL": 128, "LGN_AMD_DEC_UNFUSED": 256, "LGN_AMD_MOMENTS_SPLIT": 512,
-                 "LGN_AMD_MLP_BWD1": 1024}
+                 "LGN_AMD_MLP_BWD1": 1024, "LGN_AMD_ENC_FULL_SWEEP": 2048}
+NET_JET_IDENTITY = 4096
 ACTIVATIONS = {"leakyrelu": 0, "relu": 1, "elu": 2, "sigmoid": 3, "logsigmoid": 4, "atan": 5}
 
 
@@ -120,7 +122,8 @@
 
 
 def net_flags() -> int:
-    return sum(bit for name, bit in _NET_FLAG_ENV.items() if os.environ.get(name, "") == "1")
+    return (sum(bit for name, bit in _NET_FLAG_ENV.items() if os.environ.get(name, "") == "1") +
+            (NET_JET_IDENTITY if os.environ.get("LGN_AMD_JET_ORDER", "") == "0" else 0))
 
 
 class LossDesc(C.Structure):
```
